# wengroup/matten

Hardware: AMD Instinct MI355X
Metric: edge_tensor_products_per_sec (higher is better)
Workload: dtype f32; 1 GPU; configs[2]: synthetic fcc-64 crystals (64 atoms, cutoff 5 A, 1152 edges each), paper hparams lmax=4, eval forward backbone+out_layer, one batch per step per GPU; last conv layer run for its live outputs only (258/842 radial-weight columns: the irreps its only reader takes) -- `value` counts 4 edge-TP per edge all the same, `value_full_layers` is the rate with the full last layer; nodes_per_gpu=64000, edges_per_gpu=1152000, conv_layers=4

## Files before the change

### include/matten_hip.h

```cpp
#ifndef MATTEN_HIP_H
#define MATTEN_HIP_H

#include <stddef.h>
#include <stdint.h>

#ifdef __cplusplus
extern "C" {
#endif

typedef void* matten_stream_t;

#define MATTEN_OK 0
#define MATTEN_EINVAL (-1)
#define MATTEN_ELAUNCH (-2)
#define MATTEN_ENOMEM (-3)

int matten_abi_version(void);

#define MATTEN_RADIAL_MAX_MID 3

size_t matten_csr_workspace_bytes(int64_t n_edges, int64_t n_nodes);
int matten_csr_counting_max_avg_degree(void);
int matten_csr_build(const int64_t* edge_index, int64_t n_edges, int64_t n_nodes, int32_t* perm,
                     int32_t* rowptr, int32_t* src_sorted, void* workspace, size_t workspace_bytes,
                     int32_t* err_flag, matten_stream_t stream);

int64_t matten_csr_split_bound(int64_t n_nodes, int64_t n_edges, int64_t max_len);
int matten_csr_split(const int32_t* rowptr, int64_t n_nodes, int64_t n_edges, int64_t max_len, int32_t* vrowptr,
                     int64_t* vseg, const float* num_neigh, float* vnn, matten_stream_t stream);

size_t matten_group_workspace_bytes(int64_t n, int64_t n_keys);
int matten_group_by_key(const int64_t* key, int64_t n, int64_t n_keys, int32_t* order, int32_t* seg,
                        void* workspace, size_t workspace_bytes, int32_t* err_flag, matten_stream_t stream);

int matten_species_embed(const int64_t* atomic_numbers, int64_t n_nodes, const int64_t* z_to_index,
                         int64_t min_z, int64_t max_z, int64_t n_species, const float* weight ,
                         const float* bias , int64_t dim, int64_t* species_index, int32_t* species_i32,
                         float* node_feats, float* node_attrs, int32_t* err_flag, matten_stream_t stream);

int matten_edge_geom(const float* pos, const int64_t* edge_index, const float* edge_cell_shift,
                     const float* cell, int64_t n_cells, const int64_t* batch, const int32_t* perm,
                     int64_t n_edges, int64_t n_nodes, int lmax, int n_basis, float r_start, float r_end,
                     float* geom_sorted, float* sh_sorted, int sh_stride, float* edge_vectors, float* edge_lengths,
                     float* edge_attrs, float* edge_embedding, matten_stream_t stream);

int matten_radial_mlp(const float* geom_sorted, int64_t n_edges, int n_basis, float r_start, float r_end,
                      const float* w0p, int nb_pad, const float* w1p, const float* w2p, int hidden, int w_pad,
                      float act_cst, void* w_edge, int out_is_bf16, matten_stream_t stream);
int matten_radial_mlp_deep(const float* geom_sorted, int64_t n_edges, int n_basis, float r_start, float r_end,
                           const float* w0p, int nb_pad, const float* w_mid, int n_mid, const float* w2p, int hidden,
                           int w_pad, float act_cst, void* w_edge, int out_is_bf16, matten_stream_t stream);

int matten_tp_tile_nodes(void);
int matten_tp_paths(const float* x, int64_t d_in, const void* w_edge, int64_t w_pad, const float* sh_sorted,
                    int64_t sh_dim, const int32_t* rowptr, const int32_t* src_sorted, int64_t n_nodes,
                    const int32_t* path_entries, const int32_t* unit_start, int64_t n_entries,
                    int64_t units_per_tile, int64_t d_mid, float avg_num_neighbors, const float* num_neigh,
                    float* agg , int w_is_bf16, matten_stream_t stream);

int matten_agg_linear_max_mt(void);
int matten_agg_linear_block_chunks(void);
size_t matten_agg_linear_lds_bytes(int64_t w_stride, int64_t n_io, int64_t n_blocks);
size_t matten_agg_linear_max_lds_bytes(void);
int matten_agg_linear(const float* agg, int64_t ld, const int32_t* order, const int32_t* seg, int64_t n_species,
                      const float* wtab, int64_t w_stride, const int32_t* io_table, int64_t n_io,
                      const int32_t* blocks, int64_t n_blocks, const float* add, int64_t add_ld, int64_t d_out,
                      int64_t n_rows, float* out, matten_stream_t stream);
int matten_agg_linear_gate(const float* agg, int64_t ld, const int32_t* order, const int32_t* seg, int64_t n_species,
                           const float* wtab, int64_t w_stride, const int32_t* io_table, int64_t n_io,
                           const int32_t* blocks, int64_t n_blocks, const float* add, int64_t add_ld, int64_t d_out,
                           int64_t n_rows, const int32_t* cmeta, const float* act_cst, const float* bn_scale,
                           const float* bn_shift, int64_t d_act, float* out, matten_stream_t stream);
int matten_agg_linear_gate_sets(void);
int matten_radial_hidden(const float* geom_sorted, int64_t n_edges, int n_basis, float r_start, float r_end,
                         const float* w0p, int nb_pad, const float* w1p, int hidden, uint16_t* h2s,
                         const float* h_scale, matten_stream_t stream);
int matten_radial_hidden_multi(const float* geom_sorted, int64_t n_edges, int n_basis, float r_start, float r_end,
                               const float* const* w0p, int nb_pad, const float* const* w1p, int hidden,
                               uint16_t* const* h2s, const float* const* h_scale, int n_layers,
                               matten_stream_t stream);
int matten_radial_hidden_deep(const float* geom_sorted, int64_t n_edges, int n_basis, float r_start, float r_end,
                              const float* w0p, int nb_pad, const float* w_mid, int n_mid, int hidden, uint16_t* h2s,
                              const float* h_scale, matten_stream_t stream);
int matten_radial_hidden_multi_deep(const float* geom_sorted, int64_t n_edges, int n_basis, float r_start, float r_end,
                                    const float* const* w0p, int nb_pad, const float* const* w_mid, int n_mid, int hidden,
                                    uint16_t* const* h2s, const float* const* h_scale, int n_layers,
                                    matten_stream_t stream);
int matten_tp_fused(const float* x, int64_t d_in, const uint16_t* h2s, const float* w2p, int64_t w_pad,
                    const float* sh_sorted, int64_t sh_stride, const int32_t* rowptr, const int32_t* src_sorted,
                    int64_t n_nodes, const int32_t* group_entries, const int32_t* unit_map, int64_t n_entries,
                    int64_t units_per_tile, int64_t lds_floats_per_wave, int64_t d_mid, float avg_num_neighbors,
                    const float* num_neigh, const uint16_t* a_split, const float* a_scale_inv,
                    float* agg , matten_stream_t stream);

int matten_tp_max_cols(void);
int matten_tp_max_cols_l0(void);
int matten_tp_max_cols_l1(void);
int matten_tp_groups_hash(void);

int matten_species_linear(const float* x, int64_t d_in, const int32_t* order, const int32_t* seg, int64_t n_species,
                          const float* wp, int64_t w_stride, const int32_t* segs, int64_t n_segs, int64_t d_out,
                          const float* add, int64_t add_ld, int64_t n_rows, float* out, matten_stream_t stream);

int matten_species_linear_rows(const float* x, int64_t d_in, const int32_t* order, const int32_t* seg, int64_t n_species,
                               const float* wp, int64_t w_stride, const int32_t* segs, int64_t n_segs, int64_t d_out,
                               const float* add, int64_t add_ld, int64_t n_rows, float* out, matten_stream_t stream);

int matten_gate_bn(const float* x, int64_t d_in, const int32_t* meta, int64_t d_out, const float* act_cst,
                   const float* running_mean, const float* running_var, const float* bn_weight,
                   const float* bn_bias, float eps, int64_t n_rows, float* out, matten_stream_t stream);

int matten_segment_reduce(const float* x, int64_t dim, const int64_t* ptr, int64_t n_segments, int mean,
                          float* out, matten_stream_t stream);
int matten_segment_minmax(const float* x, int64_t dim, const int64_t* ptr, int64_t n_segments, int take_max, float* out,
                          int64_t* arg, matten_stream_t stream);
int matten_segment_minmax_bwd(const float* dy, int64_t dim, const int64_t* arg, int64_t n_segments, float* dx,
                              matten_stream_t stream);

int64_t matten_radial_mlp_bwd_small_slices(int64_t n_edges);
int64_t matten_radial_mlp_bwd_w2_ranges(int64_t n_edges, int64_t w_pad);
int matten_radial_mlp_bwd(const float* geom_sorted, int64_t n_edges, int n_basis, float r_start, float r_end,
                          const float* w0p, int nb_pad, const float* w1p, const float* w2p, int hidden, int w_pad,
                          int w_cols, const void* dw, int64_t dw_ld, int dw_is_bf16, float* h2_scratch,
                          float* part_small, float* part_w2, float scale0, float scale1, float scale2,
                          float* grad_small, float* grad_w2, matten_stream_t stream);
int64_t matten_radial_mlp_bwd_w2_ranges_deep(int64_t n_edges, int64_t w_pad, int n_mid);
int matten_radial_mlp_bwd_deep(const float* geom_sorted, int64_t n_edges, int n_basis, float r_start, float r_end,
                               const float* w0p, int nb_pad, const float* w_mid, int n_mid, const float* w2p, int hidden,
                               int w_pad, int w_cols, const void* dw, int64_t dw_ld, int dw_is_bf16, float* h2_scratch,
                               float* part_small, float* part_w2, float scale0, float scale1, float scale2,
                               float* grad_small, float* grad_w2, matten_stream_t stream);
int matten_radial_pack(const float* w0, const float* w1, const float* w2, int n_basis, int nb_pad, int w_cols, int w_pad,
                       float scale0, float scale1, float scale2, float* w0p, float* w1p, float* w2p,
                       matten_stream_t stream);
int matten_radial_pack_deep(const float* w0, const float* w_mid, int n_mid, const float* w2, int n_basis, int nb_pad,
                            int w_cols, int w_pad, float scale0, float scale1, float scale2, float* w0p, float* w_mid_p,
                            float* w2p, matten_stream_t stream);
int matten_radial_pack_cols(const float* w0, const float* w1, const float* w2, int n_basis, int nb_pad, int w_cols,
                            const int64_t* cols, int n_cols, int w_pad, float scale0, float scale1, float scale2, float* w0p,
                            float* w1p, float* w2p, matten_stream_t stream);
int matten_radial_h_scale(const float* w0, const float* w1, int n_basis, float r_start, float r_end, float act_cst,
                          float* out2, matten_stream_t stream);
int matten_radial_pack_cols_deep(const float* w0, const float* w_mid, int n_mid, const float* w2, int n_basis, int nb_pad,
                                 int w_cols, const int64_t* cols, int n_cols, int w_pad, float scale0, float scale1,
                                 float scale2, float* w0p, float* w_mid_p, float* w2p, matten_stream_t stream);
int matten_radial_h_scale_deep(const float* w0, const float* w_mid, int n_mid, int n_basis, float r_start, float r_end,
                               float act_cst, float* out2, matten_stream_t stream);
int matten_split_a_tiles(const float* w2p, int64_t w_pad, const int32_t* group_entries, int64_t n_entries,
                         const float* h_scale, uint16_t* frag, float* scale_inv, matten_stream_t stream);
int matten_gather_scale(const float* src, const int64_t* idx, const float* scale, int64_t n, int64_t scale_period,
                        int scale_by_source, float* out, const int64_t* perm2, float* out2, matten_stream_t stream);
int64_t matten_species_linear_wgrad_scratch_floats(int64_t n_rows, int64_t n_species, int64_t w_stride);

int matten_dense_rows(const float* x, int64_t n_in, const float* q, int64_t n_out, int64_t n_rows, float* out,
                      matten_stream_t stream);



int matten_tp_backward(const float* x, int64_t d_in, const void* w_edge, int64_t w_ld, const float* sh_sorted,
                       int64_t sh_stride, const int32_t* src_sorted, const int32_t* dst_sorted,
                       const int32_t* col_meta, int64_t n_cols, const uint8_t* nnz_ijk, const float* nnz_c,
                       const float* g_agg, int64_t d_mid, float avg_num_neighbors, const float* num_neigh,
                       int64_t n_edges, float* dx, void* dw, int64_t dw_ld, const int32_t* in_ptr,
                       const int32_t* in_cols, int64_t n_in, int edge_is_bf16 ,
                       matten_stream_t stream);

int matten_adam_step(float* params, const float* grads, float* exp_avg, float* exp_avg_sq, int64_t n, const float* step,
                     float lr, float beta1, float beta2, float eps, float weight_decay, matten_stream_t stream);

int matten_tp_backward_lit(const float* x, int64_t d_in, const void* w_edge, int64_t w_ld, const float* sh_sorted,
                           int64_t sh_stride, const int32_t* src_sorted, const int32_t* dst_sorted, const int32_t* blocks,
                           int64_t n_blocks, int64_t max_mul, const int32_t* paths, int64_t n_paths, const float* g_agg,
                           int64_t d_mid, float avg_num_neighbors, const float* num_neigh, int64_t n_edges, float* dx,
                           void* dw, int64_t dw_ld, int edge_is_bf16, int64_t n_nodes, const int32_t* out_ptr,
                           const int32_t* out_perm, float* dx_edges, int max_l, matten_stream_t stream);
int matten_tp_backward_lit_wfree(const float* x, int64_t d_in, const uint16_t* h2s, const uint16_t* frag, const float* w_inv,
                                 const float* sh_sorted, int64_t sh_stride, const int32_t* src_sorted,
                                 const int32_t* dst_sorted, const int32_t* blocks, int64_t n_blocks, int64_t sum_lanes,
                                 const int32_t* paths, int64_t n_paths, const float* g_agg, int64_t d_mid,
                                 float avg_num_neighbors, const float* num_neigh, int64_t n_edges, float* dx, void* dw,
                                 int64_t dw_ld, int edge_is_bf16, int64_t n_nodes, const int32_t* out_ptr,
                                 const int32_t* out_perm, float* dx_edges, int64_t lds_floats, int max_l, int max_mul,
                                 matten_stream_t stream);

int matten_species_linear_wgrad(const float* x, int64_t d_in, const float* dy, int64_t d_out, const int32_t* order,
                                const int32_t* seg, int64_t n_species, int64_t n_rows, const int32_t* segs,
                                int64_t n_segs, int64_t w_stride, float* dwp, float* scratch, matten_stream_t stream);

int matten_gate_bwd(const float* x, int64_t d_in, const int32_t* meta, int64_t d_out, const float* act_cst,
                    const float* dy, int64_t n_rows, float* dx, matten_stream_t stream);

int64_t matten_bn_scratch_floats(int64_t n_rows, int64_t dim);
int matten_bn_train_fwd(const float* x, int64_t dim, int64_t n_rows, const int32_t* col2chan, const int32_t* chan,
                        int64_t n_chan, const float* weight, const float* bias, float eps, float* mean, float* nu,
                        float* y, float* running_mean, float* running_var, float momentum, float* scratch,
                        matten_stream_t stream);
int matten_bn_train_bwd(const float* x, const float* dy, int64_t dim, int64_t n_rows, const int32_t* col2chan,
                        const int32_t* chan, int64_t n_chan, const float* mean, const float* nu, const float* weight,
                        float eps, float* A, float* B, float* dx, float* dweight, float* dbias, float* scratch,
                        matten_stream_t stream);

int matten_norm_act(const float* x, int64_t dim, int64_t n_rows, const int32_t* chan, int64_t n_chan, int act,
                    float epsilon, const float* running_mean, const float* running_var, const float* bn_weight,
                    const float* bn_bias, float bn_eps, float* y, matten_stream_t stream);
int matten_norm_act_bwd(const float* x, const float* dy, int64_t dim, int64_t n_rows, const int32_t* chan, int64_t n_chan,
                        int act, float epsilon, float* dx, matten_stream_t stream);

int64_t matten_bn_eval_bwd_scratch_floats(int64_t n_rows, int64_t n_cols);
int matten_gate_bn_eval_bwd(const float* x, int64_t d_in, const int32_t* meta, int64_t d_out, const float* act_cst,
                            const int32_t* bn_chan, int64_t n_chan, const float* running_mean, const float* running_var,
                            const float* bn_weight, float eps, const float* dy, int64_t n_rows, float* dx, float* dweight,
                            float* dbias, float* scratch, matten_stream_t stream);
int matten_norm_act_bn_eval_bwd(const float* x, const float* dy, int64_t dim, int64_t n_rows, const int32_t* chan,
                                int64_t n_chan, int act, float epsilon, const float* running_mean,
                                const float* running_var, const float* bn_weight, float bn_eps, float* dx, float* dweight,
                                float* dbias, float* scratch, matten_stream_t stream);

int matten_instance_norm_fwd(const float* x, int64_t dim, int64_t n_rows, const int64_t* seg_ptr, const int64_t* seg_of_row,
                             int64_t n_seg, const int32_t* col2chan, const int32_t* chan, int64_t n_chan,
                             const float* weight, const float* bias, float eps, float* mean, float* nu, float* y,
                             matten_stream_t stream);
int matten_instance_norm_bwd(const float* x, const float* dy, int64_t dim, int64_t n_rows, const int64_t* seg_ptr,
                             const int64_t* seg_of_row, int64_t n_seg, const int32_t* col2chan, const int32_t* chan,
                             int64_t n_chan, const float* mean, const float* nu, const float* weight, float eps, float* A,
                             float* B, float* dx, matten_stream_t stream);

int matten_segment_reduce_bwd(const float* dy, int64_t dim, const int64_t* ptr, int64_t n_segments, int mean, float* dx,
                              matten_stream_t stream);


int matten_graph_prep(const double* pos, const double* cell, const int64_t* ptr, int64_t n_crystals, double r_cut,
                      double* frac, double* bound, int64_t* batch, float* pos_f32, float* cell_f32,
                      matten_stream_t stream);
int matten_neighbor_count(const double* pos, const double* cell, const int64_t* ptr, const double* frac,
                          const double* bound, const int64_t* pair_ptr, double r_cut, int64_t n_crystals,
                          int64_t max_atoms, int32_t* counts, int32_t* counts_t, matten_stream_t stream);
int matten_neighbor_summary(const int64_t* offsets, const int64_t* pair_ptr, int64_t n_crystals, int64_t* out2,
                            matten_stream_t stream);
int matten_neighbor_fill(const double* pos, const double* cell, const int64_t* ptr, const double* frac,
                         const double* bound, const int64_t* pair_ptr, double r_cut, int64_t n_crystals,
                         int64_t max_atoms, const int64_t* offsets, int64_t n_edges, int64_t* edge_index,
                         float* edge_cell_shift, float* num_neigh, const int64_t* offsets_t, int64_t n_atoms,
                         int32_t* rowptr, int32_t* src_sorted, int32_t* perm, matten_stream_t stream);

#ifdef __cplusplus
}
#endif
#endif
```

### matten_amd/_lib.py

```python
from __future__ import annotations

import ctypes
import os
from ctypes import c_float, c_int, c_int32, c_int64, c_size_t, c_void_p

_HERE = os.path.dirname(os.path.abspath(__file__))
LIB_PATH = os.path.join(_HERE, "libmatten_hip.so")

ABI_VERSION = 46

P = c_void_p
SIGNATURES = {
    "matten_abi_version": (c_int, []),
    "matten_csr_workspace_bytes": (c_size_t, [c_int64, c_int64]),
    "matten_group_workspace_bytes": (c_size_t, [c_int64, c_int64]),
    "matten_csr_counting_max_avg_degree": (c_int, []),
    "matten_csr_build": (c_int, [P, c_int64, c_int64, P, P, P, P, c_size_t, P, P]),
    "matten_csr_split_bound": (c_int64, [c_int64, c_int64, c_int64]),
    "matten_csr_split": (c_int, [P, c_int64, c_int64, c_int64, P, P, P, P, P]),
    "matten_group_by_key": (c_int, [P, c_int64, c_int64, P, P, P, c_size_t, P, P]),
    "matten_species_embed": (c_int, [P, c_int64, P, c_int64, c_int64, c_int64, P, P, c_int64, P, P, P, P, P, P]),
    "matten_edge_geom": (c_int, [P, P, P, P, c_int64, P, P, c_int64, c_int64, c_int, c_int, c_float, c_float, P, P, c_int, P, P, P, P, P]),
    "matten_radial_mlp": (c_int, [P, c_int64, c_int, c_float, c_float, P, c_int, P, P, c_int, c_int, c_float, P, c_int, P]),
    "matten_radial_mlp_deep": (c_int, [P, c_int64, c_int, c_float, c_float, P, c_int, P, c_int, P, c_int, c_int, c_float, P, c_int,
                                       P]),
    "matten_tp_tile_nodes": (c_int, []),
    "matten_tp_paths": (c_int, [P, c_int64, P, c_int64, P, c_int64, P, P, c_int64, P, P, c_int64, c_int64, c_int64, c_float, P, P, c_int,
                                P]),
    "matten_radial_hidden_multi": (c_int, [P, c_int64, c_int, c_float, c_float, P, c_int, P, c_int, P, P, c_int, P]),
    "matten_radial_hidden_multi_deep": (c_int, [P, c_int64, c_int, c_float, c_float, P, c_int, P, c_int, c_int, P, P, c_int, P]),
    "matten_agg_linear_max_mt": (c_int, []),
    "matten_agg_linear_block_chunks": (c_int, []),
    "matten_agg_linear_lds_bytes": (c_size_t, [c_int64, c_int64, c_int64]),
    "matten_agg_linear_max_lds_bytes": (c_size_t, []),
    "matten_agg_linear": (c_int, [P, c_int64, P, P, c_int64, P, c_int64, P, c_int64, P, c_int64, P, c_int64, c_int64,
                                  c_int64, P, P]),
    "matten_agg_linear_gate": (c_int, [P, c_int64, P, P, c_int64, P, c_int64, P, c_int64, P, c_int64, P, c_int64, c_int64,
                                       c_int64, P, P, P, P, c_int64, P, P]),
    "matten_agg_linear_gate_sets": (c_int, []),
    "matten_radial_hidden": (c_int, [P, c_int64, c_int, c_float, c_float, P, c_int, P, c_int, P, P, P]),
    "matten_radial_hidden_deep": (c_int, [P, c_int64, c_int, c_float, c_float, P, c_int, P, c_int, c_int, P, P, P]),
    "matten_tp_max_cols": (c_int, []),
    "matten_tp_max_cols_l0": (c_int, []),
    "matten_tp_max_cols_l1": (c_int, []),
    "matten_tp_groups_hash": (c_int, []),
    "matten_tp_fused": (c_int, [P, c_int64, P, P, c_int64, P, c_int64, P, P, c_int64, P, P, c_int64, c_int64, c_int64, c_int64, c_float, P, P, P, P, P]),
    "matten_species_linear": (c_int, [P, c_int64, P, P, c_int64, P, c_int64, P, c_int64, c_int64, P, c_int64, c_int64, P, P]),
    "matten_species_linear_rows": (c_int, [P, c_int64, P, P, c_int64, P, c_int64, P, c_int64, c_int64, P, c_int64, c_int64, P, P]),
    "matten_radial_mlp_bwd_small_slices": (c_int64, [c_int64]),
    "matten_radial_mlp_bwd_w2_ranges": (c_int64, [c_int64, c_int64]),
    "matten_radial_mlp_bwd_w2_ranges_deep": (c_int64, [c_int64, c_int64, c_int]),
    "matten_radial_mlp_bwd": (c_int, [P, c_int64, c_int, c_float, c_float, P, c_int, P, P, c_int, c_int, c_int, P, c_int64,
                                      c_int, P, P, P, c_float, c_float, c_float, P, P, P]),
    "matten_radial_mlp_bwd_deep": (c_int, [P, c_int64, c_int, c_float, c_float, P, c_int, P, c_int, P, c_int, c_int, c_int, P,
                                           c_int64, c_int, P, P, P, c_float, c_float, c_float, P, P, P]),
    "matten_radial_pack": (c_int, [P, P, P, c_int, c_int, c_int, c_int, c_float, c_float, c_float, P, P, P, P]),
    "matten_radial_pack_deep": (c_int, [P, P, c_int, P, c_int, c_int, c_int, c_int, c_float, c_float, c_float, P, P, P, P]),
    "matten_radial_pack_cols": (c_int, [P, P, P, c_int, c_int, c_int, P, c_int, c_int, c_float, c_float, c_float, P, P, P, P]),
    "matten_radial_pack_cols_deep": (c_int, [P, P, c_int, P, c_int, c_int, c_int, P, c_int, c_int, c_float, c_float, c_float, P, P,
                                             P, P]),
    "matten_radial_h_scale": (c_int, [P, P, c_int, c_float, c_float, c_float, P, P]),
    "matten_radial_h_scale_deep": (c_int, [P, P, c_int, c_int, c_float, c_float, c_float, P, P]),
    "matten_split_a_tiles": (c_int, [P, c_int64, P, c_int64, P, P, P, P]),
    "matten_gather_scale": (c_int, [P, P, P, c_int64, c_int64, c_int, P, P, P, P]),
    "matten_species_linear_wgrad_scratch_floats": (c_int64, [c_int64, c_int64, c_int64]),
    "matten_tp_backward": (c_int, [P, c_int64, P, c_int64, P, c_int64, P, P, P, c_int64, P, P, P, c_int64, c_float, P, c_int64, P, P, c_int64,
                                   P, P, c_int64, c_int, P]),
    "matten_tp_backward_lit": (c_int, [P, c_int64, P, c_int64, P, c_int64, P, P, P, c_int64, c_int64, P, c_int64, P, c_int64, c_float,
                                       P, c_int64, P, P, c_int64, c_int, c_int64, P, P, P, c_int, P]),
    "matten_tp_backward_lit_wfree": (c_int, [P, c_int64, P, P, P, P, c_int64, P, P, P, c_int64, c_int64, P, c_int64, P, c_int64, c_float,
                                             P, c_int64, P, P, c_int64, c_int, c_int64, P, P, P, c_int64, c_int, c_int, P]),
    "matten_adam_step": (c_int, [P, P, P, P, c_int64, P, c_float, c_float, c_float, c_float, c_float, P]),
    "matten_species_linear_wgrad": (c_int, [P, c_int64, P, c_int64, P, P, c_int64, c_int64, P, c_int64, c_int64, P, P, P]),
    "matten_gate_bwd": (c_int, [P, c_int64, P, c_int64, P, P, c_int64, P, P]),
    "matten_bn_scratch_floats": (c_int64, [c_int64, c_int64]),
    "matten_bn_train_fwd": (c_int, [P, c_int64, c_int64, P, P, c_int64, P, P, c_float, P, P, P, P, P, c_float, P, P]),
    "matten_bn_train_bwd": (c_int, [P, P, c_int64, c_int64, P, P, c_int64, P, P, P, c_float, P, P, P, P, P, P, P]),
    "matten_norm_act": (c_int, [P, c_int64, c_int64, P, c_int64, c_int, c_float, P, P, P, P, c_float, P, P]),
    "matten_norm_act_bwd": (c_int, [P, P, c_int64, c_int64, P, c_int64, c_int, c_float, P, P]),
    "matten_bn_eval_bwd_scratch_floats": (c_int64, [c_int64, c_int64]),
    "matten_gate_bn_eval_bwd": (c_int, [P, c_int64, P, c_int64, P, P, c_int64, P, P, P, c_float, P, c_int64, P, P, P, P, P]),
    "matten_norm_act_bn_eval_bwd": (c_int, [P, P, c_int64, c_int64, P, c_int64, c_int, c_float, P, P, P, c_float, P, P, P, P,
                                            P]),
    "matten_instance_norm_fwd": (c_int, [P, c_int64, c_int64, P, P, c_int64, P, P, c_int64, P, P, c_float, P, P, P, P]),
    "matten_instance_norm_bwd": (c_int, [P, P, c_int64, c_int64, P, P, c_int64, P, P, c_int64, P, P, P, c_float, P, P, P, P]),
    "matten_segment_reduce_bwd": (c_int, [P, c_int64, P, c_int64, c_int, P, P]),
    "matten_graph_prep": (c_int, [P, P, P, c_int64, ctypes.c_double, P, P, P, P, P, P]),
    "matten_neighbor_count": (c_int, [P, P, P, P, P, P, ctypes.c_double, c_int64, c_int64, P, P, P]),
    "matten_neighbor_summary": (c_int, [P, P, c_int64, P, P]),
    "matten_neighbor_fill": (c_int, [P, P, P, P, P, P, ctypes.c_double, c_int64, c_int64, P, c_int64, P, P, P, P, c_int64,
                                     P, P, P, P]),
    "matten_gate_bn": (c_int, [P, c_int64, P, c_int64, P, P, P, P, P, c_float, c_int64, P, P]),
    "matten_segment_reduce": (c_int, [P, c_int64, P, c_int64, c_int, P, P]),
    "matten_segment_minmax": (c_int, [P, c_int64, P, c_int64, c_int, P, P, P]),
    "matten_segment_minmax_bwd": (c_int, [P, c_int64, P, c_int64, P, P]),
    "matten_dense_rows": (c_int, [P, c_int64, P, c_int64, c_int64, P, P]),
}

_lib = None


class MattenHipError(RuntimeError):
    pass


def load() -> ctypes.CDLL:
    global _lib
    if _lib is not None:
        return _lib
    if not os.path.exists(LIB_PATH):
        raise MattenHipError(
            f"{LIB_PATH} not found: the HIP extension is not built. matten_amd has no CPU fallback; "
            "run `make -C matten_amd/csrc` (needs hipcc, --offload-arch=gfx950)."
        )
    lib = ctypes.CDLL(LIB_PATH)
    for name, (res, args) in SIGNATURES.items():
        try:
            fn = getattr(lib, name)
        except AttributeError as e:
            raise MattenHipError(f"symbol {name} missing from {LIB_PATH}") from e
        fn.restype = res
        fn.argtypes = args
    v = lib.matten_abi_version()
    if v != ABI_VERSION:
        raise MattenHipError(f"ABI version mismatch: library {v}, python binding {ABI_VERSION}")
    _lib = lib
    return lib


_ERRORS = {-1: "MATTEN_EINVAL (bad argument)", -2: "MATTEN_ELAUNCH (HIP launch failed)", -3: "MATTEN_ENOMEM (workspace too small)"}


def check(rc: int, what: str) -> None:
    if rc != 0:
        raise MattenHipError(f"{what} failed: {_ERRORS.get(rc, rc)}")
```

### matten_amd/csrc/csr.hip

```cpp
#include <cstring>

#include <rocprim/device/device_radix_sort.hpp>
#include <rocprim/device/device_scan.hpp>

#include "common.h"

namespace {

__global__ void csr_keys_kernel(const int64_t* __restrict__ edge_index, int64_t E, int64_t N,
                                int32_t* __restrict__ keys, int32_t* __restrict__ vals, int32_t* err_flag) {
    int64_t e = (int64_t)blockIdx.x * blockDim.x + threadIdx.x;
    if (e >= E) return;
    int64_t s = edge_index[e];
    int64_t d = edge_index[E + e];
    if (s < 0 || s >= N || d < 0 || d >= N) {
        atomicOr(err_flag, 1);
        d = d < 0 ? 0 : (d >= N ? N - 1 : d);
    }
    keys[e] = (int32_t)d;
    vals[e] = (int32_t)e;
}

__global__ void csr_rowptr_kernel(const int32_t* __restrict__ keys_sorted, int64_t E, int64_t N,
                                  int32_t* __restrict__ rowptr) {
    int64_t n = (int64_t)blockIdx.x * blockDim.x + threadIdx.x;
    if (n > N) return;
    int64_t lo = 0, hi = E;
    while (lo < hi) {
        int64_t mid = (lo + hi) >> 1;
        if (keys_sorted[mid] < (int32_t)n) lo = mid + 1; else hi = mid;
    }
    rowptr[n] = (int32_t)lo;
}

__global__ void csr_src_kernel(const int64_t* __restrict__ edge_index, const int32_t* __restrict__ perm, int64_t E,
                               int64_t N, int32_t* __restrict__ src_sorted) {
    int64_t e = (int64_t)blockIdx.x * blockDim.x + threadIdx.x;
    if (e >= E) return;
    int64_t s = edge_index[perm[e]];
    s = s < 0 ? 0 : (s >= N ? N - 1 : s);
    src_sorted[e] = (int32_t)s;
}

__global__ void zero_i32_kernel(int32_t* __restrict__ p, int64_t n) {
    int64_t i = (int64_t)blockIdx.x * blockDim.x + threadIdx.x;
    if (i < n) p[i] = 0;
}

__global__ void csr_count_kernel(const int64_t* __restrict__ edge_index, int64_t E, int64_t N,
                                 int32_t* __restrict__ deg, int32_t* __restrict__ slot, int32_t* err_flag) {
    int64_t e = (int64_t)blockIdx.x * blockDim.x + threadIdx.x;
    if (e >= E) return;
    int64_t s = edge_index[e];
    int64_t d = edge_index[E + e];
    if (s < 0 || s >= N || d < 0 || d >= N) {
        atomicOr(err_flag, 1);
        d = d < 0 ? 0 : (d >= N ? N - 1 : d);
    }
    slot[e] = atomicAdd(&deg[d], 1);
}

__global__ void csr_place_kernel(const int64_t* __restrict__ edge_index, int64_t E, int64_t N,
                                 const int32_t* __restrict__ rowptr, const int32_t* __restrict__ slot,
                                 int32_t* __restrict__ ids) {
    int64_t e = (int64_t)blockIdx.x * blockDim.x + threadIdx.x;
    if (e >= E) return;
    int64_t d = edge_index[E + e];
    d = d < 0 ? 0 : (d >= N ? N - 1 : d);
    ids[rowptr[d] + slot[e]] = (int32_t)e;
}

constexpr int CSR_HUB_DEGREE = 2048;
constexpr int CSR_HUB_THREADS = 1024;
constexpr int CSR_HUB_BLOCKS = 64;

__global__ void csr_rank_kernel(const int64_t* __restrict__ edge_index, const int32_t* __restrict__ rowptr,
                                const int32_t* __restrict__ ids, int64_t E, int64_t N, int32_t* __restrict__ perm,
                                int32_t* __restrict__ src_sorted, int32_t* __restrict__ hubs) {
    const int64_t node = ((int64_t)blockIdx.x * blockDim.x + threadIdx.x) >> 4;
    if (node >= N) return;
    const int sub = threadIdx.x & 15;
    const int beg = rowptr[node], d = rowptr[node + 1] - beg;
    if (d > CSR_HUB_DEGREE) {
        if (sub == 0) hubs[atomicAdd(&hubs[N], 1)] = (int32_t)node;
        return;
    }
    for (int i = sub; i < d; i += 16) {
        const int id = ids[beg + i];
        int rank = 0;
        int j = 0;
        for (; j + 8 <= d; j += 8) {
            int v[8];
#pragma unroll
            for (int q = 0; q < 8; ++q) v[q] = ids[beg + j + q];
#pragma unroll
            for (int q = 0; q < 8; ++q) rank += v[q] < id;
        }
        for (; j < d; ++j) rank += ids[beg + j] < id;
        perm[beg + rank] = id;
        int64_t s = edge_index[id];
        s = s < 0 ? 0 : (s >= N ? N - 1 : s);
        src_sorted[beg + rank] = (int32_t)s;
    }
}

__global__ __launch_bounds__(CSR_HUB_THREADS) void csr_hub_kernel(const int64_t* __restrict__ edge_index,
                                                                  const int32_t* __restrict__ rowptr, int32_t* ids,
                                                                  int64_t N, int32_t* __restrict__ perm,
                                                                  int32_t* __restrict__ src_sorted,
                                                                  const int32_t* __restrict__ hubs) {
    const int n_hubs = hubs[N];
    for (int h = blockIdx.x; h < n_hubs; h += gridDim.x) {
        const int node = hubs[h];
        const int beg = rowptr[node], d = rowptr[node + 1] - beg;
        int32_t* a = ids + beg;
        for (int64_t k = 2; (k >> 1) < d; k <<= 1) {
            for (int64_t j = k >> 1; j > 0; j >>= 1) {
                const int64_t m = (j == (k >> 1)) ? k - 1 : j;
                for (int64_t i = threadIdx.x; i < d; i += CSR_HUB_THREADS) {
                    const int64_t l = i ^ m;
                    if (l > i && l < d) {
                        const int32_t x = a[i], y = a[l];
                        if (y < x) a[i] = y, a[l] = x;
                    }
                }
                __syncthreads();
            }
        }
        for (int64_t i = threadIdx.x; i < d; i += CSR_HUB_THREADS) {
            const int32_t id = a[i];
            perm[beg + i] = id;
            int64_t s = edge_index[id];
            s = s < 0 ? 0 : (s >= N ? N - 1 : s);
            src_sorted[beg + i] = (int32_t)s;
        }
        __syncthreads();
    }
}

__global__ void group_keys_kernel(const int64_t* __restrict__ key, int64_t n, int64_t n_keys,
                                  int32_t* __restrict__ keys, int32_t* __restrict__ vals, int32_t* err_flag) {
    int64_t i = (int64_t)blockIdx.x * blockDim.x + threadIdx.x;
    if (i >= n) return;
    int64_t k = key[i];
    if (k < 0 || k >= n_keys) {
        atomicOr(err_flag, 1);
        k = k < 0 ? 0 : n_keys - 1;
    }
    keys[i] = (int32_t)k;
    vals[i] = (int32_t)i;
}

constexpr int GROUP_COUNTING_MAX_KEYS = 256;
constexpr int GROUP_WAVES = 4;

__device__ __forceinline__ int group_key_of(const int64_t* __restrict__ key, int64_t i, int64_t n, int64_t n_keys,
                                            int32_t* err_flag) {
    if (i >= n) return -1;
    int64_t k = key[i];
    if (k < 0 || k >= n_keys) {
        atomicOr(err_flag, 1);
        k = k < 0 ? 0 : n_keys - 1;
    }
    return (int)k;
}

__global__ __launch_bounds__(GROUP_WAVES * 64) void group_hist_kernel(const int64_t* __restrict__ key, int64_t n,
                                                                      int64_t n_keys, int64_t n_runs,
                                                                      int32_t* __restrict__ cnt, int32_t* err_flag) {
    __shared__ int h[GROUP_WAVES][GROUP_COUNTING_MAX_KEYS];
    const int wv = threadIdx.x >> 6, lane = threadIdx.x & 63;
    const int64_t run = (int64_t)blockIdx.x * GROUP_WAVES + wv;
    for (int kk = lane; kk < n_keys; kk += 64) h[wv][kk] = 0;
    __builtin_amdgcn_wave_barrier();
    const int k = group_key_of(key, run * 64 + lane, n, n_keys, err_flag);
    if (k >= 0) atomicAdd(&h[wv][k], 1);
    __builtin_amdgcn_s_waitcnt(0xc07f);
    __builtin_amdgcn_wave_barrier();
    if (run < n_runs)
        for (int kk = lane; kk < n_keys; kk += 64) cnt[(int64_t)kk * n_runs + run] = h[wv][kk];
}

__global__ __launch_bounds__(GROUP_WAVES * 64) void group_place_kernel(const int64_t* __restrict__ key, int64_t n,
                                                                       int64_t n_keys, int64_t n_runs,
                                                                       const int32_t* __restrict__ offs,
                                                                       int32_t* __restrict__ order,
                                                                       int32_t* __restrict__ seg, int32_t* err_flag) {
    const int lane = threadIdx.x & 63;
    const int64_t i = (int64_t)blockIdx.x * blockDim.x + threadIdx.x;
    const int64_t run = i >> 6;
    if (i <= n_keys) seg[i] = i < n_keys ? offs[i * n_runs] : (int32_t)n;
    const int k = group_key_of(key, i, n, n_keys, err_flag);
    unsigned long long todo = __ballot(k >= 0);
    int rank = 0;
    while (todo) {
        const int kf = __shfl(k, __ffsll((long long)todo) - 1);
        const unsigned long long m = __ballot(k == kf);
        if (k == kf) rank = __popcll(m & ((1ull << lane) - 1ull));
        todo &= ~m;
    }
    if (k >= 0) order[offs[(int64_t)k * n_runs + run] + rank] = (int32_t)i;
}

inline size_t align256(size_t x) { return (x + 255) & ~(size_t)255; }

inline int key_bits(int64_t N) {
    int b = 1;
    while (((int64_t)1 << b) < N && b < 31) ++b;
    return b;
}

}

__global__ __launch_bounds__(1024) void csr_split_kernel(const int* __restrict__ rowptr, int N, int max_len, int nv_bound,
                                                         int* __restrict__ vrowptr, int64_t* __restrict__ vseg,
                                                         const float* __restrict__ num_neigh, float* __restrict__ vnn) {
    __shared__ int sh[1024];
    __shared__ int carry_s;
    const int t = threadIdx.x;
    if (t == 0) carry_s = 0;
    __syncthreads();
    const int E = rowptr[N];
    for (int base = 0; base < N; base += 1024) {
        const int n = base + t;
        int beg = 0, k = 0, d = 0;
        if (n < N) {
            beg = rowptr[n];
            d = rowptr[n + 1] - beg;
            k = max(1, (d + max_len - 1) / max_len);
        }
        sh[t] = k;
        __syncthreads();
        for (int off = 1; off < 1024; off <<= 1) {
            const int v = t >= off ? sh[t - off] : 0;
            __syncthreads();
            sh[t] += v;
            __syncthreads();
        }
        const int carry = carry_s;
        const int first = carry + sh[t] - k;
        if (n < N) {
            vseg[n] = first;
            for (int i = 0; i < k; ++i) {
                const int v = first + i;
                if (v < nv_bound) {
                    vrowptr[v] = beg + (int)((int64_t)i * d / k);
                    if (vnn) vnn[v] = num_neigh[n];
                }
            }
        }
        __syncthreads();
        if (t == 1023) carry_s = carry + sh[1023];
        __syncthreads();
    }
    const int nv = min(carry_s, nv_bound);
    if (t == 0) vseg[N] = nv;
    for (int v = nv + t; v <= nv_bound; v += 1024) {
        vrowptr[v] = E;
        if (vnn && v < nv_bound) vnn[v] = 1.0f;
    }
}

extern "C" size_t matten_csr_workspace_bytes(int64_t E, int64_t N) {
    if (E < 0 || N < 0) return 0;
    size_t tmp = 0;
    int32_t* p = nullptr;
    (void)rocprim::radix_sort_pairs(nullptr, tmp, p, p, p, p, (size_t)(E > 0 ? E : 1), 0, key_bits(N), 0, false);
    size_t scan_tmp = 0;
    (void)rocprim::exclusive_scan(nullptr, scan_tmp, p, p, 0, (size_t)(N + 1), rocprim::plus<int32_t>());
    return 3 * align256((size_t)(E > 0 ? E : 1) * sizeof(int32_t)) + align256(tmp) + align256((size_t)(N + 1) * sizeof(int32_t)) +
           align256(scan_tmp) + 256;
}

extern "C" size_t matten_group_workspace_bytes(int64_t n, int64_t n_keys) {
    if (n < 0 || n_keys <= 0) return 0;
    size_t need = matten_csr_workspace_bytes(n, n_keys);
    if (n_keys <= GROUP_COUNTING_MAX_KEYS) {
        const size_t table = (size_t)n_keys * (size_t)((n + 63) / 64 + 1);
        size_t scan_tmp = 0;
        int32_t* p = nullptr;
        (void)rocprim::exclusive_scan(nullptr, scan_tmp, p, p, 0, table, rocprim::plus<int32_t>());
        const size_t counting = 2 * align256(table * sizeof(int32_t)) + align256(scan_tmp) + 256;
        if (counting > need) need = counting;
    }
    return need;
}

constexpr int64_t CSR_COUNTING_MAX_AVG_DEGREE = 64;

extern "C" int matten_csr_counting_max_avg_degree(void) { return (int)CSR_COUNTING_MAX_AVG_DEGREE; }

extern "C" int matten_csr_build(const int64_t* edge_index, int64_t E, int64_t N, int32_t* perm, int32_t* rowptr,
                                int32_t* src_sorted, void* workspace, size_t workspace_bytes, int32_t* err_flag,
                                matten_stream_t stream_) {
    hipStream_t stream = (hipStream_t)stream_;
    if (E < 0 || N < 0 || N >= ((int64_t)1 << 31) || E >= ((int64_t)1 << 31)) return MATTEN_EINVAL;
    if (!rowptr || !err_flag) return MATTEN_EINVAL;
    if (E == 0) {
        zero_i32_kernel<<<(unsigned)matten_cdiv(N + 1, 256), 256, 0, stream>>>(rowptr, N + 1);
        MATTEN_LAUNCH_CHECK();
        return MATTEN_OK;
    }
    if (!edge_index || !perm || !src_sorted || !workspace) return MATTEN_EINVAL;
    size_t need = matten_csr_workspace_bytes(E, N);
    if (workspace_bytes < need) return MATTEN_ENOMEM;

    char* ws = (char*)workspace;
    size_t seg = align256((size_t)E * sizeof(int32_t));
    int32_t* keys_in = (int32_t*)ws;
    int32_t* keys_out = (int32_t*)(ws + seg);
    int32_t* vals_in = (int32_t*)(ws + 2 * seg);
    void* tmp = ws + 3 * seg;
    size_t tmp_bytes = workspace_bytes - 3 * seg;

    const int T = 256;
    if (N > 0 && E <= CSR_COUNTING_MAX_AVG_DEGREE * N) {
        int32_t* ids = (int32_t*)ws;
        int32_t* slot = (int32_t*)(ws + seg);
        int32_t* deg = (int32_t*)(ws + 2 * seg);
        const size_t deg_bytes = align256((size_t)(N + 1) * sizeof(int32_t));
        void* scan_tmp = ws + 2 * seg + deg_bytes;
        size_t scan_bytes = workspace_bytes - 2 * seg - deg_bytes;
        zero_i32_kernel<<<(unsigned)matten_cdiv(N + 1, T), T, 0, stream>>>(deg, N + 1);
        MATTEN_LAUNCH_CHECK();
        csr_count_kernel<<<(unsigned)matten_cdiv(E, T), T, 0, stream>>>(edge_index, E, N, deg, slot, err_flag);
        MATTEN_LAUNCH_CHECK();
        if (rocprim::exclusive_scan(scan_tmp, scan_bytes, deg, rowptr, 0, (size_t)(N + 1), rocprim::plus<int32_t>(),
                                    stream) != hipSuccess)
            return MATTEN_ELAUNCH;
        csr_place_kernel<<<(unsigned)matten_cdiv(E, T), T, 0, stream>>>(edge_index, E, N, rowptr, slot, ids);
        MATTEN_LAUNCH_CHECK();
        csr_rank_kernel<<<(unsigned)matten_cdiv(N * 16, T), T, 0, stream>>>(edge_index, rowptr, ids, E, N, perm,
                                                                           src_sorted, deg);
        MATTEN_LAUNCH_CHECK();
        if (E > CSR_HUB_DEGREE) {
            const int64_t max_hubs = E / CSR_HUB_DEGREE;
            csr_hub_kernel<<<(unsigned)(max_hubs < CSR_HUB_BLOCKS ? max_hubs : CSR_HUB_BLOCKS), CSR_HUB_THREADS, 0,
                             stream>>>(edge_index, rowptr, ids, N, perm, src_sorted, deg);
            MATTEN_LAUNCH_CHECK();
        }
        return MATTEN_OK;
    }
    csr_keys_kernel<<<(unsigned)matten_cdiv(E, T), T, 0, stream>>>(edge_index, E, N, keys_in, vals_in, err_flag);
    MATTEN_LAUNCH_CHECK();
    if (rocprim::radix_sort_pairs(tmp, tmp_bytes, keys_in, keys_out, vals_in, perm, (size_t)E, 0, key_bits(N), stream,
                                  false) != hipSuccess)
        return MATTEN_ELAUNCH;
    csr_rowptr_kernel<<<(unsigned)matten_cdiv(N + 1, T), T, 0, stream>>>(keys_out, E, N, rowptr);
    MATTEN_LAUNCH_CHECK();
    csr_src_kernel<<<(unsigned)matten_cdiv(E, T), T, 0, stream>>>(edge_index, perm, E, N, src_sorted);
    MATTEN_LAUNCH_CHECK();
    return MATTEN_OK;
}

extern "C" int matten_group_by_key(const int64_t* key, int64_t n, int64_t n_keys, int32_t* order, int32_t* seg,
                                   void* workspace, size_t workspace_bytes, int32_t* err_flag, matten_stream_t stream_) {
    hipStream_t stream = (hipStream_t)stream_;
    if (n < 0 || n_keys <= 0 || n_keys >= ((int64_t)1 << 31) || n >= ((int64_t)1 << 31)) return MATTEN_EINVAL;
    if (!seg || !err_flag) return MATTEN_EINVAL;
    if (n == 0) {
        zero_i32_kernel<<<(unsigned)matten_cdiv(n_keys + 1, 256), 256, 0, stream>>>(seg, n_keys + 1);
        MATTEN_LAUNCH_CHECK();
        return MATTEN_OK;
    }
    if (!key || !order || !workspace) return MATTEN_EINVAL;
    if (workspace_bytes < matten_group_workspace_bytes(n, n_keys)) return MATTEN_ENOMEM;
    char* ws = (char*)workspace;
    if (n_keys <= GROUP_COUNTING_MAX_KEYS) {
        const int64_t n_runs = (n + 63) / 64;
        const size_t table = (size_t)n_keys * (size_t)n_runs;
        const size_t tb = align256((size_t)n_keys * (size_t)(n_runs + 1) * sizeof(int32_t));
        int32_t* cnt = (int32_t*)ws;
        int32_t* offs = (int32_t*)(ws + tb);
        void* scan_tmp = ws + 2 * tb;
        size_t scan_bytes = workspace_bytes - 2 * tb;
        const int TB = GROUP_WAVES * 64;
        group_hist_kernel<<<(unsigned)matten_cdiv(n_runs, GROUP_WAVES), TB, 0, stream>>>(key, n, n_keys, n_runs, cnt,
                                                                                        err_flag);
        MATTEN_LAUNCH_CHECK();
        if (rocprim::exclusive_scan(scan_tmp, scan_bytes, cnt, offs, 0, table, rocprim::plus<int32_t>(), stream) !=
            hipSuccess)
            return MATTEN_ELAUNCH;
        const int64_t threads = n > n_keys + 1 ? n : n_keys + 1;
        group_place_kernel<<<(unsigned)matten_cdiv(threads, TB), TB, 0, stream>>>(key, n, n_keys, n_runs, offs, order,
                                                                                 seg, err_flag);
        MATTEN_LAUNCH_CHECK();
        return MATTEN_OK;
    }
    size_t sg = align256((size_t)n * sizeof(int32_t));
    int32_t* keys_in = (int32_t*)ws;
    int32_t* keys_out = (int32_t*)(ws + sg);
    int32_t* vals_in = (int32_t*)(ws + 2 * sg);
    void* tmp = ws + 3 * sg;
    size_t tmp_bytes = workspace_bytes - 3 * sg;
    const int T = 256;
    group_keys_kernel<<<(unsigned)matten_cdiv(n, T), T, 0, stream>>>(key, n, n_keys, keys_in, vals_in, err_flag);
    MATTEN_LAUNCH_CHECK();
    if (rocprim::radix_sort_pairs(tmp, tmp_bytes, keys_in, keys_out, vals_in, order, (size_t)n, 0, key_bits(n_keys),
                                  stream, false) != hipSuccess)
        return MATTEN_ELAUNCH;
    csr_rowptr_kernel<<<(unsigned)matten_cdiv(n_keys + 1, T), T, 0, stream>>>(keys_out, n, n_keys, seg);
    MATTEN_LAUNCH_CHECK();
    return MATTEN_OK;
}

extern "C" int64_t matten_csr_split_bound(int64_t n_nodes, int64_t n_edges, int64_t max_len) {
    return max_len > 0 ? n_nodes + n_edges / max_len : n_nodes;
}

extern "C" int matten_csr_split(const int32_t* rowptr, int64_t n_nodes, int64_t n_edges, int64_t max_len, int32_t* vrowptr,
                                int64_t* vseg, const float* num_neigh, float* vnn, matten_stream_t stream_) {
    if (n_nodes < 0 || n_edges < 0 || max_len <= 0 || n_nodes >= ((int64_t)1 << 30) || n_edges >= ((int64_t)1 << 31))
        return MATTEN_EINVAL;
    if (!rowptr || !vrowptr || !vseg || ((num_neigh == nullptr) != (vnn == nullptr))) return MATTEN_EINVAL;
    const int64_t bound = matten_csr_split_bound(n_nodes, n_edges, max_len);
    if (bound >= ((int64_t)1 << 31)) return MATTEN_EINVAL;
    csr_split_kernel<<<1, 1024, 0, (hipStream_t)stream_>>>(rowptr, (int)n_nodes, (int)max_len, (int)bound, vrowptr, vseg,
                                                          num_neigh, vnn);
    MATTEN_LAUNCH_CHECK();
    return MATTEN_OK;
}
```

### matten_amd/csrc/edge.hip

```cpp
#include "common.h"
#include "sh.h"

namespace {

constexpr int SH_TILE_RS = 36;

template <int LMAX>
__global__ __launch_bounds__(256) void edge_geom_kernel(const float* __restrict__ pos, const int64_t* __restrict__ edge_index,
                                 const float* __restrict__ shift, const float* __restrict__ cell, int64_t n_cells,
                                 const int64_t* __restrict__ batch, const int32_t* __restrict__ perm, int64_t E,
                                 int64_t N, int n_basis, float r_start, float r_end, float4* __restrict__ geom_sorted,
                                 float* __restrict__ sh_sorted, int sh_stride, float* __restrict__ edge_vectors,
                                 float* __restrict__ edge_lengths, float* __restrict__ edge_attrs,
                                 float* __restrict__ edge_embedding) {
    constexpr int SH = (LMAX + 1) * (LMAX + 1);
    __shared__ __attribute__((aligned(16))) float sh_tile[4 * 64 * SH_TILE_RS];
    const int64_t e_raw = (int64_t)blockIdx.x * blockDim.x + threadIdx.x;
    if (e_raw - (threadIdx.x & 63) >= E) return;
    const bool live = e_raw < E;
    const int64_t e = live ? e_raw : E - 1;
    int64_t o = perm ? (int64_t)perm[e] : e;
    int64_t i = edge_index[o];
    int64_t j = edge_index[E + o];
    i = i < 0 ? 0 : (i >= N ? N - 1 : i);
    j = j < 0 ? 0 : (j >= N ? N - 1 : j);
    float vx = pos[3 * j + 0] - pos[3 * i + 0];
    float vy = pos[3 * j + 1] - pos[3 * i + 1];
    float vz = pos[3 * j + 2] - pos[3 * i + 2];
    if (cell) {
        int64_t b = (n_cells > 1 && batch) ? batch[i] : 0;
        b = b < 0 ? 0 : (b >= n_cells ? n_cells - 1 : b);
        const float* c = cell + 9 * b;
        float s0 = shift[3 * o + 0], s1 = shift[3 * o + 1], s2 = shift[3 * o + 2];
        vx += s0 * c[0] + s1 * c[3] + s2 * c[6];
        vy += s0 * c[1] + s1 * c[4] + s2 * c[7];
        vz += s0 * c[2] + s1 * c[5] + s2 * c[8];
    }
    float len = sqrtf(vx * vx + vy * vy + vz * vz);
    if (live) geom_sorted[e] = make_float4(vx, vy, vz, len);

    float y[SH];
    matten::real_sh<LMAX>(vx, vy, vz, len, y);
    if (sh_stride == 32) {
        float* tile = sh_tile + (threadIdx.x >> 6) * (64 * SH_TILE_RS);
        const int lane = threadIdx.x & 63;
#pragma unroll
        for (int q = 0; q < 8; ++q)
            *reinterpret_cast<float4*>(tile + lane * SH_TILE_RS + 4 * q) =
                make_float4(4 * q < SH ? y[4 * q < SH ? 4 * q : 0] : 0.0f,
                            4 * q + 1 < SH ? y[4 * q + 1 < SH ? 4 * q + 1 : 0] : 0.0f,
                            4 * q + 2 < SH ? y[4 * q + 2 < SH ? 4 * q + 2 : 0] : 0.0f,
                            4 * q + 3 < SH ? y[4 * q + 3 < SH ? 4 * q + 3 : 0] : 0.0f);
        __builtin_amdgcn_s_waitcnt(0xc07f);
        __builtin_amdgcn_wave_barrier();
        const int64_t e0 = e_raw - lane;
        const int64_t n_here = E - e0 < 64 ? E - e0 : 64;
        float4* dst = reinterpret_cast<float4*>(sh_sorted + e0 * 32);
#pragma unroll
        for (int i = 0; i < 8; ++i) {
            const int f = i * 64 + lane;
            if ((f >> 3) < n_here)
                dst[f] = *reinterpret_cast<const float4*>(tile + (f >> 3) * SH_TILE_RS + 4 * (f & 7));
        }
    } else if (live) {
#pragma unroll
        for (int k = 0; k < SH; ++k) sh_sorted[e * sh_stride + k] = y[k];
        for (int k = SH; k < sh_stride; ++k) sh_sorted[e * sh_stride + k] = 0.0f;
    }
    if (!live) return;

    if (edge_vectors) {
        edge_vectors[3 * o + 0] = vx;
        edge_vectors[3 * o + 1] = vy;
        edge_vectors[3 * o + 2] = vz;
    }
    if (edge_lengths) edge_lengths[o] = len;
    if (edge_attrs) {
#pragma unroll
        for (int k = 0; k < SH; ++k) edge_attrs[o * SH + k] = y[k];
    }
    if (edge_embedding) {
        for (int k = 0; k < n_basis; ++k)
            edge_embedding[o * n_basis + k] = matten::bessel_basis(len, k, n_basis, r_start, r_end);
    }
}

__global__ void species_embed_kernel(const int64_t* __restrict__ Z, int64_t N, const int64_t* __restrict__ lut,
                                     int64_t min_z, int64_t max_z, int64_t S, const float* __restrict__ W,
                                     const float* __restrict__ b, int64_t dim, int64_t* __restrict__ species_index,
                                     int32_t* __restrict__ species_i32, float* __restrict__ feats,
                                     float* __restrict__ attrs, int32_t* err_flag) {
    int64_t n = (int64_t)blockIdx.x * blockDim.y + threadIdx.y;
    if (n >= N) return;
    int64_t z = Z[n];
    int64_t idx = -1;
    if (z < min_z || z > max_z) {
        if (threadIdx.x == 0) atomicOr(err_flag, 2);
    } else {
        idx = lut[z - min_z];
        if (idx < 0 || idx >= S) {
            if (threadIdx.x == 0) atomicOr(err_flag, 4);
            idx = -1;
        }
    }
    if (threadIdx.x == 0) {
        if (species_index) species_index[n] = idx;
        if (species_i32) species_i32[n] = (int32_t)(idx < 0 ? 0 : idx);
    }
    int64_t s = idx < 0 ? 0 : idx;
    for (int64_t d = threadIdx.x; d < dim; d += blockDim.x) feats[n * dim + d] = W[d * S + s] + b[d];
    if (attrs)
        for (int64_t c = threadIdx.x; c < S; c += blockDim.x) attrs[n * S + c] = (c == idx) ? 1.0f : 0.0f;
}

}

extern "C" int matten_species_embed(const int64_t* atomic_numbers, int64_t n_nodes, const int64_t* z_to_index,
                                    int64_t min_z, int64_t max_z, int64_t n_species, const float* weight,
                                    const float* bias, int64_t dim, int64_t* species_index, int32_t* species_i32,
                                    float* node_feats, float* node_attrs, int32_t* err_flag,
                                    matten_stream_t stream_) {
    hipStream_t stream = (hipStream_t)stream_;
    if (n_nodes < 0 || dim <= 0 || n_species <= 0) return MATTEN_EINVAL;
    if (n_nodes == 0) return MATTEN_OK;
    if (!atomic_numbers || !z_to_index || !weight || !bias || !node_feats || !err_flag) return MATTEN_EINVAL;
    dim3 block(16, 16);
    species_embed_kernel<<<(unsigned)matten_cdiv(n_nodes, 16), block, 0, stream>>>(
        atomic_numbers, n_nodes, z_to_index, min_z, max_z, n_species, weight, bias, dim, species_index, species_i32,
        node_feats, node_attrs, err_flag);
    MATTEN_LAUNCH_CHECK();
    return MATTEN_OK;
}

extern "C" int matten_edge_geom(const float* pos, const int64_t* edge_index, const float* edge_cell_shift,
                                const float* cell, int64_t n_cells, const int64_t* batch, const int32_t* perm,
                                int64_t n_edges, int64_t n_nodes, int lmax, int n_basis, float r_start, float r_end,
                                float* geom_sorted, float* sh_sorted, int sh_stride, float* edge_vectors, float* edge_lengths,
                                float* edge_attrs, float* edge_embedding, matten_stream_t stream_) {
    hipStream_t stream = (hipStream_t)stream_;
    if (n_edges < 0 || n_nodes < 0 || (n_edges > 0 && n_nodes == 0) || lmax < 0 || lmax > 4 || n_basis < 0 || sh_stride < (lmax + 1) * (lmax + 1)) return MATTEN_EINVAL;
    if (n_edges == 0) return MATTEN_OK;
    if (!pos || !edge_index || !geom_sorted || !sh_sorted) return MATTEN_EINVAL;
    if (cell && !edge_cell_shift) return MATTEN_EINVAL;
    const int T = 256;
    unsigned grid = (unsigned)matten_cdiv(n_edges, T);
#define LAUNCH(L)                                                                                              \
    edge_geom_kernel<L><<<grid, T, 0, stream>>>(pos, edge_index, edge_cell_shift, cell, n_cells, batch, perm,  \
                                                n_edges, n_nodes, n_basis, r_start, r_end, (float4*)geom_sorted, \
                                                sh_sorted, sh_stride, edge_vectors, edge_lengths, edge_attrs, edge_embedding)
    switch (lmax) {
        case 0: LAUNCH(0); break;
        case 1: LAUNCH(1); break;
        case 2: LAUNCH(2); break;
        case 3: LAUNCH(3); break;
        default: LAUNCH(4); break;
    }
#undef LAUNCH
    MATTEN_LAUNCH_CHECK();
    return MATTEN_OK;
}
```

### matten_amd/nn/_nequip.py

```python
from typing import Union

import torch

from .. import ops
from ..data.irreps import DataKey, ModuleIrreps
from ..o3 import Irreps


def with_batch(data: DataKey.Type) -> DataKey.Type:
    if DataKey.BATCH not in data:
        pos = data[DataKey.POSITIONS]
        data[DataKey.BATCH] = torch.zeros(len(pos), dtype=torch.long, device=pos.device)
    return data


def ensure_graph(data: DataKey.Type, err=None) -> DataKey.Type:
    if DataKey.AMD_ROWPTR not in data:
        n_nodes = data[DataKey.POSITIONS].shape[0]
        perm, rowptr, src, err = ops.csr_build(data[DataKey.EDGE_INDEX], n_nodes, err=err)
        data[DataKey.AMD_PERM], data[DataKey.AMD_ROWPTR], data[DataKey.AMD_SRC] = perm, rowptr, src
        data["_amd_csr_err"] = err
    return data


def ensure_edge_geometry(data: DataKey.Type, lmax: int = None, want_vectors=False, want_lengths=False,
                         want_attrs=False, want_embedding=False) -> DataKey.Type:
    have = DataKey.AMD_GEOM in data
    missing = (
        (want_vectors and DataKey.EDGE_VECTORS not in data)
        or (want_lengths and DataKey.EDGE_LENGTH not in data)
        or (want_attrs and DataKey.EDGE_ATTRS not in data)
        or (want_embedding and DataKey.EDGE_EMBEDDING not in data)
    )
    if have and not missing:
        return data
    ensure_graph(data)
    if lmax is None:
        lmax = int(data["_amd_lmax"]) if "_amd_lmax" in data else 0
    data["_amd_lmax"] = lmax
    nb, r0, r1 = 0, 0.0, 1.0
    if DataKey.AMD_RBF in data:
        nb, r0, r1 = data[DataKey.AMD_RBF].tolist()
        nb = int(nb)
    out = ops.edge_geom(
        data[DataKey.POSITIONS], data[DataKey.EDGE_INDEX], data.get(DataKey.EDGE_CELL_SHIFT),
        data.get(DataKey.CELL), data.get(DataKey.BATCH), data[DataKey.AMD_PERM], lmax, nb, r0, r1,
        want_vectors=want_vectors, want_lengths=want_lengths, want_attrs=want_attrs,
        want_embedding=want_embedding and nb > 0,
    )
    data[DataKey.AMD_GEOM], data[DataKey.AMD_SH] = out["geom_sorted"], out["sh_sorted"]
    for key, name in ((DataKey.EDGE_VECTORS, "edge_vectors"), (DataKey.EDGE_LENGTH, "edge_lengths"),
                      (DataKey.EDGE_ATTRS, "edge_attrs"), (DataKey.EDGE_EMBEDDING, "edge_embedding")):
        if out[name] is not None:
            data[key] = out[name]
    return data


def ensure_training_edge_tensors(data: DataKey.Type) -> DataKey.Type:
    if "_amd_dst_sorted" not in data:
        ensure_edge_geometry(data)
        perm = data[DataKey.AMD_PERM].long()
        data["_amd_dst_sorted"] = data[DataKey.EDGE_INDEX][1][perm].to(torch.int32).contiguous()
        src = data[DataKey.AMD_SRC].long()
        pairs = torch.stack([src, src])
        out_perm, out_ptr, _, _ = ops.csr_build(pairs, int(data[DataKey.POSITIONS].shape[0]))
        data["_amd_out_csr"] = (out_ptr, out_perm)
    return data


def with_edge_vectors(data: DataKey.Type, with_lengths: bool = True) -> DataKey.Type:
    return ensure_edge_geometry(data, want_vectors=True, want_lengths=with_lengths)


class SphericalHarmonicEdgeAttrs(ModuleIrreps, torch.nn.Module):
    out_field: str

    def __init__(
        self,
        irreps_edge_sh: Union[int, str, Irreps],
        edge_sh_normalization: str = "component",
        edge_sh_normalize: bool = True,
        irreps_in=None,
        out_field: str = DataKey.EDGE_ATTRS,
        materialize: bool = False,
    ):
        super().__init__()
        self.out_field = out_field
        if isinstance(irreps_edge_sh, int):
            self.irreps_edge_sh = Irreps.spherical_harmonics(irreps_edge_sh)
        else:
            self.irreps_edge_sh = Irreps(irreps_edge_sh)
        lmax = len(self.irreps_edge_sh) - 1
        if self.irreps_edge_sh != Irreps.spherical_harmonics(lmax) or lmax > 4:
            raise NotImplementedError(f"edge SH must be 0e+1o+...+lmax (lmax<=4), got {self.irreps_edge_sh}")
        if edge_sh_normalization != "component" or not edge_sh_normalize:
            raise NotImplementedError("only normalize=True, normalization='component' (the reference default)")
        self.lmax = lmax
        self.materialize = materialize
        self.init_irreps(irreps_in=irreps_in, irreps_out={out_field: self.irreps_edge_sh})

    def forward(self, data: DataKey.Type) -> DataKey.Type:
        ensure_edge_geometry(data, lmax=self.lmax, want_vectors=self.materialize, want_attrs=self.materialize)
        if self.materialize and self.out_field != DataKey.EDGE_ATTRS:
            data[self.out_field] = data[DataKey.EDGE_ATTRS]
        return data
```

### matten_amd/nn/embedding.py

```python
from typing import Dict, List, Tuple

import numpy as np
import torch

from .. import ops
from ..data.irreps import DataKey, ModuleIrreps
from ..o3 import Irreps


class _AtomicNumberToIndex(torch.nn.Module):

    def __init__(self, allowed_atomic_numbers: List[int]):
        super().__init__()
        allowed = torch.as_tensor(sorted(allowed_atomic_numbers), dtype=torch.long)
        lut = torch.full((int(allowed.max() - allowed.min()) + 1,), -1, dtype=torch.long)
        lut[allowed - allowed.min()] = torch.arange(len(allowed), dtype=torch.long)
        self.register_buffer("_min_Z", allowed.min())
        self.register_buffer("_max_Z", allowed.max())
        self.register_buffer("_num_species", torch.as_tensor(len(allowed)))
        self.register_buffer("_Z_to_index", lut)
        self._host = (int(allowed.min()), int(allowed.max()), len(allowed))
        self._allowed = [int(z) for z in allowed]

    @property
    def num_species(self):
        return self._num_species

    def raise_for_flags(self, flags: int, atomic_numbers: torch.Tensor):
        if flags & 2:
            raise RuntimeError(
                "Invalid atomic numbers. Expect atomic numbers to be in the range "
                f"[{self._host[0]}, {self._host[1]}], but got min {int(atomic_numbers.min())} "
                f"and max {int(atomic_numbers.max())}"
            )
        if flags & 4:
            z = atomic_numbers.cpu()
            for i, n in enumerate(z.tolist()):
                if n not in self._allowed:
                    raise RuntimeError(
                        f"Expect atomic numbers to be in {self._allowed}, "
                        f"got invalid atomic numbers `{n}` for data point `{i}`."
                    )

    def forward(self, atomic_numbers: torch.Tensor) -> torch.Tensor:
        lo, hi, _ = self._host
        if atomic_numbers.min() < lo or atomic_numbers.max() > hi:
            self.raise_for_flags(2, atomic_numbers)
        index = self._Z_to_index[atomic_numbers - lo]
        if index.min() < 0:
            self.raise_for_flags(4, atomic_numbers)
        return index


class SpeciesEmbedding(ModuleIrreps, torch.nn.Module):
    def __init__(
        self,
        irreps_in: Dict[str, Irreps] = None,
        embedding_dim: int = 16,
        num_species: int = None,
        allowed_species: List[int] = None,
        out_fields: Tuple[str] = (DataKey.NODE_ATTRS, DataKey.NODE_FEATURES),
        use_atom_feats: bool = False,
        atom_feats_dim: int = None,
        materialize: bool = False,
        check_species: bool = True,
    ):
        super().__init__()
        if allowed_species is not None and num_species is not None:
            raise ValueError("allowed_species and num_species cannot both be provided.")
        if allowed_species is None:
            raise NotImplementedError("matten_amd needs `allowed_species` (every shipped config provides it)")
        if use_atom_feats and atom_feats_dim is None:
            raise ValueError("`atom_feats_dim` must be provided if `use_atom_feats` is True.")
        self.use_atom_feats = use_atom_feats
        self.embedding_dim = embedding_dim
        self.out_fields = out_fields
        self.materialize = materialize
        self.check_species = check_species
        self.atomic_number_to_index = _AtomicNumberToIndex(allowed_species)
        self.num_species = len(allowed_species)
        self.init_irreps(
            irreps_in,
            {DataKey.NODE_ATTRS: Irreps(f"{self.num_species}x0e"),
             DataKey.NODE_FEATURES: Irreps(f"{embedding_dim + (atom_feats_dim if use_atom_feats else 0)}x0e")},
        )
        self.linear = torch.nn.Linear(self.num_species, embedding_dim)

    def finish_checks(self) -> None:
        pending, self._pending = getattr(self, "_pending", None), None
        if pending is None:
            return
        ev, host, Z, n_nodes = pending
        ev.synchronize()
        self._raise_for(host.tolist(), Z, n_nodes)

    def _raise_for(self, flags, Z, n_nodes) -> None:
        if flags[0]:
            self.atomic_number_to_index.raise_for_flags(flags[0], Z)
        if flags[1] & 1:
            rng = f"[0, {n_nodes})" if n_nodes is not None else "the batch's node range"
            raise IndexError(f"edge_index holds node ids outside {rng} (a malformed batch)")

    def raise_for_last_flags(self, n_nodes=None) -> None:
        flags_dev = getattr(self, "_last_flags", None)
        if flags_dev is None:
            return
        self._raise_for(flags_dev.tolist(), self._last_Z, n_nodes)

    def forward(self, data: DataKey.Type) -> DataKey.Type:
        a2i = self.atomic_number_to_index
        lo, hi, S = a2i._host
        if DataKey.SPECIES_INDEX in data:
            Z = data[DataKey.SPECIES_INDEX]
            lut = torch.arange(S, dtype=torch.int64, device=Z.device)
            lo, hi = 0, S - 1
            provided = True
        elif DataKey.ATOMIC_NUMBERS in data:
            Z, lut, provided = data[DataKey.ATOMIC_NUMBERS], a2i._Z_to_index, False
        else:
            raise ValueError("Nothing in `data` to encode. Need either species_index or atomic_numbers")
        flags_dev = torch.zeros(3, dtype=torch.int32, device=Z.device)
        sidx, s32, feats, attrs, _ = ops.species_embed(
            Z, lut, lo, hi, S, self.linear.weight, self.linear.bias, want_attrs=self.materialize, err=flags_dev[0:1]
        )
        if DataKey.EDGE_INDEX in data:
            from ._nequip import ensure_graph

            built_here = DataKey.AMD_ROWPTR not in data
            csr_err = ensure_graph(data, err=flags_dev[1:2]).get("_amd_csr_err")
            if not built_here and csr_err is not None:
                flags_dev[1:2] = csr_err
        order, seg, _ = ops.group_by_key(sidx, S, err=flags_dev[2:3])
        self._last_flags, self._last_Z = flags_dev, Z
        n_nodes = data[DataKey.POSITIONS].shape[0] if DataKey.POSITIONS in data else None
        if self.check_species == "deferred":
            self.finish_checks()
            host = torch.empty(3, dtype=torch.int32, pin_memory=True)
            host.copy_(flags_dev, non_blocking=True)
            ev = torch.cuda.Event()
            ev.record(torch.cuda.current_stream(Z.device))
            self._pending = (ev, host, Z, n_nodes)
        elif self.check_species:
            self.raise_for_last_flags(n_nodes)
        if not provided:
            data[DataKey.SPECIES_INDEX] = sidx
        data[DataKey.AMD_SPECIES] = (order, seg)
        data[DataKey.AMD_SPECIES_I32] = s32
        if attrs is not None:
            data[DataKey.NODE_ATTRS] = attrs
        if torch.is_grad_enabled() and self.linear.weight.requires_grad:
            from ..autograd import SpeciesEmbedFn

            if self.__dict__.get("_wgrad_segs") is None:
                from ._tables import DeviceTables

                dim = self.linear.weight.shape[0]
                self.__dict__["_wgrad_segs"] = DeviceTables(segs=np.array([[0, 1, 1, 0, dim, 0, 0, 0]], dtype=np.int32))
            feats = SpeciesEmbedFn.apply(self.linear.weight, self.linear.bias, feats, (order, seg),
                                         self._wgrad_segs.get("segs", feats.device))
        if self.use_atom_feats:
            extra = data["atom_feats"]
            if extra.dim() != 2 or extra.shape[0] != feats.shape[0]:
                raise ValueError(f"atom_feats must be [n_atoms, atom_feats_dim], got {tuple(extra.shape)}")
            feats = torch.cat([feats, extra.to(feats.dtype)], dim=1)
        data[DataKey.NODE_FEATURES] = feats
        return data


class EdgeLengthEmbedding(ModuleIrreps, torch.nn.Module):
    REQUIRED_KEYS_IRREPS_IN = [DataKey.POSITIONS, DataKey.EDGE_INDEX]

    def __init__(
        self,
        irreps_in: Dict[str, Irreps] = None,
        out_field: str = DataKey.EDGE_EMBEDDING,
        num_basis: int = 10,
        start: float = 0.0,
        end: float = 5.0,
        basis: str = "bessel",
        cutoff: bool = True,
        materialize: bool = False,
    ):
        super().__init__()
        if basis != "bessel" or not cutoff:
            raise NotImplementedError("matten_amd implements the Bessel basis with cutoff (all shipped configs)")
        self.num_basis, self.start, self.end, self.basis, self.cutoff = num_basis, start, end, basis, cutoff
        self.out_field = out_field
        self.materialize = materialize
        self.init_irreps(irreps_in, irreps_out={out_field: Irreps(f"{num_basis}x0e")})

    def forward(self, data: DataKey.Type) -> DataKey.Type:
        from ._nequip import ensure_edge_geometry

        data[DataKey.AMD_RBF] = torch.tensor([self.num_basis, self.start, self.end], dtype=torch.float64)
        if self.materialize:
            ensure_edge_geometry(data, want_lengths=True, want_embedding=True)
        return data
```

### matten_amd/ops.py

```python
from __future__ import annotations

from typing import Optional, Tuple

import os

import numpy as np

import torch

from . import _lib
from .nn._tables import bump_weights_epoch


_EVENTS = None
_EVENTS_ONLY = None


def enable_event_timing(flag: bool = True, only=None) -> None:
    global _EVENTS, _EVENTS_ONLY
    _EVENTS = {} if flag else None
    _EVENTS_ONLY = tuple(only) if (flag and only) else None


def event_timings_ms():
    if _EVENTS is None:
        return {}
    return {k: [a.elapsed_time(b) for a, b in v] for k, v in _EVENTS.items()}


class _timed:
    def __init__(self, name: str):
        self.name = name

    def __enter__(self):
        self.on = _EVENTS is not None and (_EVENTS_ONLY is None or self.name.startswith(_EVENTS_ONLY))
        if self.on:
            self.a = torch.cuda.Event(enable_timing=True)
            self.a.record(torch.cuda.current_stream())
        return self

    def __exit__(self, *exc):
        if self.on and _EVENTS is not None:
            b = torch.cuda.Event(enable_timing=True)
            b.record(torch.cuda.current_stream())
            _EVENTS.setdefault(self.name, []).append((self.a, b))
        return False


SH_STRIDE = 32


def _ptr(t: Optional[torch.Tensor]):
    return None if t is None else t.data_ptr()


_raw_stream = getattr(torch._C, "_cuda_getCurrentRawStream", None)


def _stream() -> int:
    if _raw_stream is not None:
        return _raw_stream(torch.cuda.current_device())
    return torch.cuda.current_stream().cuda_stream


def _need(t: torch.Tensor, dtype, name: str) -> torch.Tensor:
    if not isinstance(t, torch.Tensor):
        raise TypeError(f"{name}: expected a tensor, got {type(t)}")
    if not t.is_cuda:
        raise _lib.MattenHipError(
            f"{name} is on {t.device}: matten_amd runs on MI355X only (no CPU fallback). Move the batch to cuda."
        )
    if t.dtype != dtype:
        raise TypeError(f"{name}: expected dtype {dtype}, got {t.dtype}")
    return t if t.is_contiguous() else t.contiguous()


def _need_rows(t: torch.Tensor, dtype, name: str) -> torch.Tensor:
    if isinstance(t, torch.Tensor) and t.dim() == 2 and t.stride(1) == 1 and t.stride(0) >= t.shape[1] and t.is_cuda \
            and t.dtype == dtype:
        return t
    return _need(t, dtype, name)


def _err_flag(err, dev) -> torch.Tensor:
    if err is None:
        return torch.zeros(1, dtype=torch.int32, device=dev)
    if err.dtype != torch.int32 or err.numel() != 1 or err.device != dev:
        raise ValueError("err must be an int32 tensor of one element on the inputs' device")
    return err


def csr_build(edge_index: torch.Tensor, n_nodes: int, err: torch.Tensor = None) -> Tuple[torch.Tensor, torch.Tensor, torch.Tensor, torch.Tensor]:
    lib = _lib.load()
    edge_index = _need(edge_index, torch.int64, "edge_index")
    E = edge_index.shape[1]
    dev = edge_index.device
    perm = torch.empty(E, dtype=torch.int32, device=dev)
    rowptr = torch.empty(n_nodes + 1, dtype=torch.int32, device=dev)
    src = torch.empty(E, dtype=torch.int32, device=dev)
    err = _err_flag(err, dev)
    nbytes = lib.matten_csr_workspace_bytes(E, n_nodes)
    ws = torch.empty(max(nbytes, 1), dtype=torch.uint8, device=dev)
    _lib.check(
        lib.matten_csr_build(_ptr(edge_index), E, n_nodes, _ptr(perm), _ptr(rowptr), _ptr(src), _ptr(ws), nbytes,
                             _ptr(err), _stream()),
        "matten_csr_build",
    )
    return perm, rowptr, src, err


def csr_split(rowptr: torch.Tensor, n_edges: int, max_len: int, num_neigh: torch.Tensor = None):
    lib = _lib.load()
    rowptr = _need(rowptr, torch.int32, "rowptr")
    N = rowptr.shape[0] - 1
    bound = int(lib.matten_csr_split_bound(N, n_edges, max_len))
    dev = rowptr.device
    vrowptr = torch.empty(bound + 1, dtype=torch.int32, device=dev)
    vseg = torch.empty(N + 1, dtype=torch.int64, device=dev)
    vnn = None
    if num_neigh is not None:
        num_neigh = _need(num_neigh, torch.float32, "num_neigh")
        vnn = torch.empty(bound, dtype=torch.float32, device=dev)
    _lib.check(lib.matten_csr_split(_ptr(rowptr), N, n_edges, max_len, _ptr(vrowptr), _ptr(vseg), _ptr(num_neigh), _ptr(vnn),
                                    _stream()), "matten_csr_split")
    return vrowptr, vseg, vnn


def group_by_key(key: torch.Tensor, n_keys: int, err: torch.Tensor = None) -> Tuple[torch.Tensor, torch.Tensor, torch.Tensor]:
    lib = _lib.load()
    key = _need(key, torch.int64, "key")
    n = key.shape[0]
    dev = key.device
    order = torch.empty(n, dtype=torch.int32, device=dev)
    seg = torch.empty(n_keys + 1, dtype=torch.int32, device=dev)
    err = _err_flag(err, dev)
    nbytes = lib.matten_group_workspace_bytes(n, n_keys)
    ws = torch.empty(max(nbytes, 1), dtype=torch.uint8, device=dev)
    _lib.check(lib.matten_group_by_key(_ptr(key), n, n_keys, _ptr(order), _ptr(seg), _ptr(ws), nbytes, _ptr(err),
                                       _stream()), "matten_group_by_key")
    return order, seg, err


def species_embed(atomic_numbers, z_to_index, min_z: int, max_z: int, n_species: int, weight, bias,
                  want_attrs: bool = False, err: torch.Tensor = None):
    lib = _lib.load()
    Z = _need(atomic_numbers, torch.int64, "atomic_numbers")
    lut = _need(z_to_index, torch.int64, "_Z_to_index")
    W = _need(weight, torch.float32, "linear.weight")
    b = _need(bias, torch.float32, "linear.bias")
    N, dim = Z.shape[0], W.shape[0]
    dev = Z.device
    sidx = torch.empty(N, dtype=torch.int64, device=dev)
    s32 = torch.empty(N, dtype=torch.int32, device=dev)
    feats = torch.empty(N, dim, dtype=torch.float32, device=dev)
    attrs = torch.empty(N, n_species, dtype=torch.float32, device=dev) if want_attrs else None
    err = _err_flag(err, dev)
    _lib.check(
        lib.matten_species_embed(_ptr(Z), N, _ptr(lut), min_z, max_z, n_species, _ptr(W), _ptr(b), dim, _ptr(sidx),
                                 _ptr(s32), _ptr(feats), _ptr(attrs), _ptr(err), _stream()),
        "matten_species_embed",
    )
    return sidx, s32, feats, attrs, err


def edge_geom(pos, edge_index, edge_cell_shift, cell, batch, perm, lmax: int, n_basis: int = 0, r_start: float = 0.0,
              r_end: float = 1.0, want_vectors=False, want_lengths=False, want_attrs=False, want_embedding=False):
    lib = _lib.load()
    pos = _need(pos, torch.float32, "pos")
    edge_index = _need(edge_index, torch.int64, "edge_index")
    E = edge_index.shape[1]
    dev = pos.device
    n_cells = 0
    if cell is not None:
        cell = _need(cell, torch.float32, "cell").reshape(-1, 3, 3)
        n_cells = cell.shape[0]
        edge_cell_shift = _need(edge_cell_shift, torch.float32, "edge_cell_shift")
        if n_cells > 1:
            batch = _need(batch, torch.int64, "batch")
    sh_dim = (lmax + 1) ** 2
    geom = torch.empty(E, 4, dtype=torch.float32, device=dev)
    sh = torch.empty(E, SH_STRIDE, dtype=torch.float32, device=dev)
    out = {"geom_sorted": geom, "sh_sorted": sh}
    ev = torch.empty(E, 3, dtype=torch.float32, device=dev) if want_vectors else None
    el = torch.empty(E, dtype=torch.float32, device=dev) if want_lengths else None
    ea = torch.empty(E, sh_dim, dtype=torch.float32, device=dev) if want_attrs else None
    ee = torch.empty(E, n_basis, dtype=torch.float32, device=dev) if want_embedding else None
    _lib.check(
        lib.matten_edge_geom(_ptr(pos), _ptr(edge_index), _ptr(edge_cell_shift), _ptr(cell), n_cells, _ptr(batch),
                             _ptr(perm), E, pos.shape[0], lmax, n_basis, r_start, r_end, _ptr(geom), _ptr(sh), SH_STRIDE, _ptr(ev),
                             _ptr(el),
                             _ptr(ea), _ptr(ee), _stream()),
        "matten_edge_geom",
    )
    out.update(edge_vectors=ev, edge_lengths=el, edge_attrs=ea, edge_embedding=ee)
    return out


def _edge_dtype(t: torch.Tensor, name: str) -> torch.Tensor:
    if not isinstance(t, torch.Tensor) or t.dtype not in (torch.float32, torch.bfloat16):
        raise TypeError(f"{name}: expected an fp32 or bf16 tensor")
    return _need(t, t.dtype, name)


def radial_mlp(geom_sorted, n_basis: int, r_start: float, r_end: float, w0p, w1p, w2p, out_dtype=torch.float32) -> torch.Tensor:
    lib = _lib.load()
    geom_sorted = _need(geom_sorted, torch.float32, "geom_sorted")
    w0p, w1p, w2p = (_need(w, torch.float32, n) for w, n in ((w0p, "w0p"), (w1p, "w1p"), (w2p, "w2p")))
    E = geom_sorted.shape[0]
    nb_pad, hidden = w0p.shape
    w_pad = w2p.shape[1]
    if out_dtype not in (torch.float32, torch.bfloat16):
        raise TypeError("radial_mlp: out_dtype must be fp32 or bf16")
    out = torch.empty(E, w_pad, dtype=out_dtype, device=geom_sorted.device)
    with _timed(f"radial_mlp/w_pad={w_pad}"):
        rc = lib.matten_radial_mlp(_ptr(geom_sorted), E, n_basis, r_start, r_end, _ptr(w0p), nb_pad, _ptr(w1p),
                                   _ptr(w2p), hidden, w_pad, 1.0, _ptr(out), int(out_dtype == torch.bfloat16), _stream())
    _lib.check(rc, "matten_radial_mlp")
    return out


def radial_pack(w0, w1, w2, scales):
    lib = _lib.load()
    w0, w1, w2 = (_need(w, torch.float32, n) for w, n in ((w0, "layer0.weight"), (w1, "layer1.weight"), (w2, "layer2.weight")))
    nb, h = w0.shape
    W = w2.shape[1]
    nb_pad, w_pad = (nb + 3) // 4 * 4, (W + 15) // 16 * 16
    dev = w0.device
    w0p = torch.empty(nb_pad, h, dtype=torch.float32, device=dev)
    w1p = torch.empty(h, h, dtype=torch.float32, device=dev)
    w2p = torch.empty(h, w_pad, dtype=torch.float32, device=dev)
    _lib.check(lib.matten_radial_pack(_ptr(w0), _ptr(w1), _ptr(w2), nb, nb_pad, W, w_pad, float(scales[0]), float(scales[1]),
                                      float(scales[2]), _ptr(w0p), _ptr(w1p), _ptr(w2p), _stream()), "matten_radial_pack")
    return w0p, w1p, w2p


def fused_operands(w0, w1, w2, scales, cols, group_entries, n_tiles: int, r_start: float, r_end: float, act_cst: float):
    lib = _lib.load()
    w0, w1, w2 = (_need(w, torch.float32, n) for w, n in ((w0, "layer0.weight"), (w1, "layer1.weight"), (w2, "layer2.weight")))
    cols = _need(cols, torch.int64, "fused_cols")
    group_entries = _need(group_entries, torch.int32, "group_entries")
    nb, h = w0.shape
    W, n_cols = w2.shape[1], cols.numel()
    nb_pad, w_pad = (nb + 3) // 4 * 4, (n_cols + 15) // 16 * 16 + 16
    dev = w0.device
    w0p = torch.empty(nb_pad, h, dtype=torch.float32, device=dev)
    w1p = torch.empty(h, h, dtype=torch.float32, device=dev)
    w2p = torch.empty(h, w_pad, dtype=torch.float32, device=dev)
    hs = torch.empty(2, dtype=torch.float32, device=dev)
    n_ent = group_entries.shape[0]
    frag = torch.empty(n_tiles, 64, 16, dtype=torch.float16, device=dev)
    inv = torch.empty(n_ent, dtype=torch.float32, device=dev)
    st = _stream()
    _lib.check(lib.matten_radial_pack_cols(_ptr(w0), _ptr(w1), _ptr(w2), nb, nb_pad, W, _ptr(cols), n_cols, w_pad,
                                           float(scales[0]), float(scales[1]), float(scales[2]), _ptr(w0p), _ptr(w1p),
                                           _ptr(w2p), st), "matten_radial_pack_cols")
    _lib.check(lib.matten_radial_h_scale(_ptr(w0), _ptr(w1), nb, float(r_start), float(r_end), float(act_cst), _ptr(hs), st),
               "matten_radial_h_scale")
    _lib.check(lib.matten_split_a_tiles(_ptr(w2p), w_pad, _ptr(group_entries), n_ent, _ptr(hs), _ptr(frag), _ptr(inv), st),
               "matten_split_a_tiles")
    return w0p, w1p, w2p, hs, frag, inv


RADIAL_MAX_MID = 3


def _mid(w_mid, name: str):
    if not isinstance(w_mid, torch.Tensor) or w_mid.dim() != 3 or tuple(w_mid.shape[1:]) != (32, 32):
        raise ValueError(f"{name}: expected [n_mid, 32, 32]")
    n_mid = w_mid.shape[0]
    if n_mid > RADIAL_MAX_MID:
        raise ValueError(f"{name}: at most {RADIAL_MAX_MID} middle layers (invariant_layers <= {RADIAL_MAX_MID + 1})")
    return (_need(w_mid, torch.float32, name) if n_mid else None), n_mid


def radial_mlp_deep(geom_sorted, n_basis: int, r_start: float, r_end: float, w0p, w_mid, w2p,
                    out_dtype=torch.float32) -> torch.Tensor:
    lib = _lib.load()
    geom_sorted = _need(geom_sorted, torch.float32, "geom_sorted")
    w0p, w2p = _need(w0p, torch.float32, "w0p"), _need(w2p, torch.float32, "w2p")
    w_mid, n_mid = _mid(w_mid, "w_mid")
    E = geom_sorted.shape[0]
    nb_pad, hidden = w0p.shape
    w_pad = w2p.shape[1]
    if out_dtype not in (torch.float32, torch.bfloat16):
        raise TypeError("radial_mlp: out_dtype must be fp32 or bf16")
    out = torch.empty(E, w_pad, dtype=out_dtype, device=geom_sorted.device)
    with _timed(f"radial_mlp/w_pad={w_pad}"):
        rc = lib.matten_radial_mlp_deep(_ptr(geom_sorted), E, n_basis, r_start, r_end, _ptr(w0p), nb_pad, _ptr(w_mid), n_mid,
                                        _ptr(w2p), hidden, w_pad, 1.0, _ptr(out), int(out_dtype == torch.bfloat16), _stream())
    _lib.check(rc, "matten_radial_mlp_deep")
    return out


def radial_pack_deep(w0, w_mid, w2, scales):
    lib = _lib.load()
    w0, w2 = _need(w0, torch.float32, "layer0.weight"), _need(w2, torch.float32, "last layer weight")
    w_mid, n_mid = _mid(w_mid, "middle layer weights")
    nb, h = w0.shape
    W = w2.shape[1]
    nb_pad, w_pad = (nb + 3) // 4 * 4, (W + 15) // 16 * 16
    dev = w0.device
    w0p = torch.empty(nb_pad, h, dtype=torch.float32, device=dev)
    wmp = torch.empty(n_mid, h, h, dtype=torch.float32, device=dev)
    w2p = torch.empty(h, w_pad, dtype=torch.float32, device=dev)
    _lib.check(lib.matten_radial_pack_deep(_ptr(w0), _ptr(w_mid), n_mid, _ptr(w2), nb, nb_pad, W, w_pad, float(scales[0]),
                                           float(scales[1]), float(scales[2]), _ptr(w0p), _ptr(wmp) if n_mid else None,
                                           _ptr(w2p), _stream()), "matten_radial_pack_deep")
    return w0p, wmp, w2p


def radial_h_scale_deep(w0, w_mid, r_start: float, r_end: float, act_cst: float) -> torch.Tensor:
    lib = _lib.load()
    w0 = _need(w0, torch.float32, "layer0.weight")
    w_mid, n_mid = _mid(w_mid, "middle layer weights")
    hs = torch.empty(2, dtype=torch.float32, device=w0.device)
    _lib.check(lib.matten_radial_h_scale_deep(_ptr(w0), _ptr(w_mid), n_mid, w0.shape[0], float(r_start), float(r_end),
                                              float(act_cst), _ptr(hs), _stream()), "matten_radial_h_scale_deep")
    return hs


def fused_operands_deep(w0, w_mid, w2, scales, cols, group_entries, n_tiles: int, r_start: float, r_end: float,
                        act_cst: float):
    lib = _lib.load()
    w0, w2 = _need(w0, torch.float32, "layer0.weight"), _need(w2, torch.float32, "last layer weight")
    w_mid, n_mid = _mid(w_mid, "middle layer weights")
    cols = _need(cols, torch.int64, "fused_cols")
    group_entries = _need(group_entries, torch.int32, "group_entries")
    nb, h = w0.shape
    W, n_cols = w2.shape[1], cols.numel()
    nb_pad, w_pad = (nb + 3) // 4 * 4, (n_cols + 15) // 16 * 16 + 16
    dev = w0.device
    w0p = torch.empty(nb_pad, h, dtype=torch.float32, device=dev)
    wmp = torch.empty(n_mid, h, h, dtype=torch.float32, device=dev)
    w2p = torch.empty(h, w_pad, dtype=torch.float32, device=dev)
    hs = torch.empty(2, dtype=torch.float32, device=dev)
    n_ent = group_entries.shape[0]
    frag = torch.empty(n_tiles, 64, 16, dtype=torch.float16, device=dev)
    inv = torch.empty(n_ent, dtype=torch.float32, device=dev)
    st = _stream()
    _lib.check(lib.matten_radial_pack_cols_deep(_ptr(w0), _ptr(w_mid), n_mid, _ptr(w2), nb, nb_pad, W, _ptr(cols), n_cols,
                                                w_pad, float(scales[0]), float(scales[1]), float(scales[2]), _ptr(w0p),
                                                _ptr(wmp) if n_mid else None, _ptr(w2p), st), "matten_radial_pack_cols_deep")
    _lib.check(lib.matten_radial_h_scale_deep(_ptr(w0), _ptr(w_mid), n_mid, nb, float(r_start), float(r_end), float(act_cst),
                                              _ptr(hs), st), "matten_radial_h_scale_deep")
    _lib.check(lib.matten_split_a_tiles(_ptr(w2p), w_pad, _ptr(group_entries), n_ent, _ptr(hs), _ptr(frag), _ptr(inv), st),
               "matten_split_a_tiles")
    return w0p, wmp, w2p, hs, frag, inv


def radial_mlp_bwd_deep(geom_sorted, n_basis: int, r_start: float, r_end: float, w0p, w_mid, w2p, w_cols: int, dw,
                        scales=(1.0, 1.0, 1.0)):
    lib = _lib.load()
    geom_sorted = _need(geom_sorted, torch.float32, "geom_sorted")
    w0p, w2p = _need(w0p, torch.float32, "w0p"), _need(w2p, torch.float32, "w2p")
    w_mid, n_mid = _mid(w_mid, "w_mid")
    if dw.dtype not in (torch.float32, torch.bfloat16):
        raise TypeError("dw must be fp32 or bf16")
    dw = _need(dw, dw.dtype, "dw")
    E = geom_sorted.shape[0]
    nb_pad, hidden = w0p.shape
    w_pad = w2p.shape[1]
    dev = geom_sorted.device
    small_len = nb_pad * hidden + n_mid * hidden * hidden
    if E == 0:
        return w0p.new_zeros(nb_pad, hidden), w0p.new_zeros(n_mid, hidden, hidden), w2p.new_zeros(hidden, w_pad)
    n_small, n_rng = lib.matten_radial_mlp_bwd_small_slices(E), lib.matten_radial_mlp_bwd_w2_ranges_deep(E, w_pad, n_mid)
    h2 = torch.empty(E, hidden, dtype=torch.float32, device=dev)
    part_small = torch.empty(max(n_small, 1), small_len, dtype=torch.float32, device=dev)
    part_w2 = torch.empty(max(n_rng, 1), hidden, w_pad, dtype=torch.float32, device=dev)
    small = torch.empty(small_len, dtype=torch.float32, device=dev)
    d2 = torch.empty(hidden, w_pad, dtype=torch.float32, device=dev)
    with _timed(f"radial_mlp_bwd/w_pad={w_pad}"):
        rc = lib.matten_radial_mlp_bwd_deep(_ptr(geom_sorted), E, n_basis, r_start, r_end, _ptr(w0p), nb_pad, _ptr(w_mid),
                                            n_mid, _ptr(w2p), hidden, w_pad, int(w_cols), _ptr(dw), dw.shape[1],
                                            int(dw.dtype == torch.bfloat16), _ptr(h2), _ptr(part_small), _ptr(part_w2),
                                            float(scales[0]), float(scales[1]), float(scales[2]), _ptr(small), _ptr(d2),
                                            _stream())
    _lib.check(rc, "matten_radial_mlp_bwd_deep")
    return small[: nb_pad * hidden].reshape(nb_pad, hidden), small[nb_pad * hidden:].reshape(n_mid, hidden, hidden), d2


def gather_scale(src, idx, scale, scale_by_source: bool = False, perm2=None):
    lib = _lib.load()
    src = _need(src, torch.float32, "src")
    idx = _need(idx, torch.int64, "idx")
    scale = _need(scale, torch.float32, "scale")
    out = torch.empty(idx.shape, dtype=torch.float32, device=src.device)
    out2 = None
    if perm2 is not None:
        perm2 = _need(perm2, torch.int64, "perm2")
        out2 = torch.empty(idx.shape, dtype=torch.float32, device=src.device)
    _lib.check(lib.matten_gather_scale(_ptr(src), _ptr(idx), _ptr(scale), idx.numel(), scale.numel(), int(scale_by_source),
                                       _ptr(out), _ptr(perm2), _ptr(out2), _stream()), "matten_gather_scale")
    return out if perm2 is None else (out, out2)


def radial_mlp_bwd(geom_sorted, n_basis: int, r_start: float, r_end: float, w0p, w1p, w2p, w_cols: int, dw,
                   scales=(1.0, 1.0, 1.0)):
    lib = _lib.load()
    geom_sorted = _need(geom_sorted, torch.float32, "geom_sorted")
    w0p, w1p, w2p = (_need(w, torch.float32, n) for w, n in ((w0p, "w0p"), (w1p, "w1p"), (w2p, "w2p")))
    if dw.dtype not in (torch.float32, torch.bfloat16):
        raise TypeError("dw must be fp32 or bf16")
    dw = _need(dw, dw.dtype, "dw")
    E = geom_sorted.shape[0]
    nb_pad, hidden = w0p.shape
    w_pad = w2p.shape[1]
    dev = geom_sorted.device
    n_small, n_rng = lib.matten_radial_mlp_bwd_small_slices(E), lib.matten_radial_mlp_bwd_w2_ranges(E, w_pad)
    h2 = torch.empty(E, hidden, dtype=torch.float32, device=dev)
    part_small = torch.empty(max(n_small, 1), nb_pad * hidden + hidden * hidden, dtype=torch.float32, device=dev)
    part_w2 = torch.empty(max(n_rng, 1), hidden, w_pad, dtype=torch.float32, device=dev)
    if E == 0:
        return w0p.new_zeros(nb_pad, hidden), w1p.new_zeros(hidden, hidden), w2p.new_zeros(hidden, w_pad)
    small = torch.empty(nb_pad * hidden + hidden * hidden, dtype=torch.float32, device=dev)
    d2 = torch.empty(hidden, w_pad, dtype=torch.float32, device=dev)
    with _timed(f"radial_mlp_bwd/w_pad={w_pad}"):
        rc = lib.matten_radial_mlp_bwd(_ptr(geom_sorted), E, n_basis, r_start, r_end, _ptr(w0p), nb_pad, _ptr(w1p),
                                       _ptr(w2p), hidden, w_pad, int(w_cols), _ptr(dw), dw.shape[1],
                                       int(dw.dtype == torch.bfloat16), _ptr(h2), _ptr(part_small), _ptr(part_w2),
                                       float(scales[0]), float(scales[1]), float(scales[2]), _ptr(small), _ptr(d2),
                                       _stream())
    _lib.check(rc, "matten_radial_mlp_bwd")
    return small[: nb_pad * hidden].reshape(nb_pad, hidden), small[nb_pad * hidden:].reshape(hidden, hidden), d2


def tp_paths(x, w_edge, sh_sorted, rowptr, src_sorted, entries, unit_start, units_per_tile: int, d_mid: int,
             avg_num_neighbors: float, num_neigh=None) -> torch.Tensor:
    lib = _lib.load()
    from .plan import TP_TILE_NODES

    if lib.matten_tp_tile_nodes() != TP_TILE_NODES:
        raise _lib.MattenHipError("plan.TP_TILE_NODES does not match the library's node tile")
    x = _need(x, torch.float32, "node_features")
    w_edge = _edge_dtype(w_edge, "w_edge")
    sh_sorted = _need(sh_sorted, torch.float32, "sh_sorted")
    N, d_in = rowptr.shape[0] - 1, x.shape[1]
    if num_neigh is not None:
        num_neigh = _need(num_neigh, torch.float32, "num_neigh")
    agg = torch.empty(N, d_mid, dtype=torch.float32, device=x.device)
    with _timed(f"tp_scatter/d_mid={d_mid}"):
        rc = lib.matten_tp_paths(_ptr(x), d_in, _ptr(w_edge), w_edge.shape[1], _ptr(sh_sorted), sh_sorted.shape[1],
                                 _ptr(rowptr), _ptr(src_sorted), N, _ptr(entries), _ptr(unit_start),
                                 entries.shape[0], units_per_tile, d_mid, float(avg_num_neighbors or 0.0),
                                 _ptr(num_neigh), _ptr(agg), int(w_edge.dtype == torch.bfloat16), _stream())
    _lib.check(rc, "matten_tp_paths")
    return agg


def split_hidden(h2p: torch.Tensor) -> torch.Tensor:
    tiny = 2.0 ** -14
    hi = torch.where(h2p.abs() < tiny, torch.zeros_like(h2p), h2p.half().float())
    lo = (h2p - hi) * 2048.0
    lo = torch.where(lo.abs() < tiny, torch.zeros_like(lo), lo)
    return torch.stack([hi.half(), lo.half()], dim=1).contiguous()


def radial_hidden(geom_sorted, n_basis: int, r_start: float, r_end: float, w0p, w1p, h_scale=None) -> torch.Tensor:
    lib = _lib.load()
    geom_sorted = _need(geom_sorted, torch.float32, "geom_sorted")
    w0p, w1p = _need(w0p, torch.float32, "w0p"), _need(w1p, torch.float32, "w1p")
    E = geom_sorted.shape[0]
    h2p = torch.empty(E, 2, 32, dtype=torch.float16, device=geom_sorted.device)
    with _timed("radial_hidden"):
        if h_scale is not None:
            h_scale = _need(h_scale, torch.float32, "h_scale")
        rc = lib.matten_radial_hidden(_ptr(geom_sorted), E, n_basis, r_start, r_end, _ptr(w0p), w0p.shape[0],
                                      _ptr(w1p), w0p.shape[1], _ptr(h2p), _ptr(h_scale), _stream())
    _lib.check(rc, "matten_radial_hidden")
    return h2p


def radial_hidden_multi(geom_sorted, n_basis: int, r_start: float, r_end: float, w0ps, w1ps, h_scales=None):
    import ctypes

    lib = _lib.load()
    geom_sorted = _need(geom_sorted, torch.float32, "geom_sorted")
    w0ps = [_need(w, torch.float32, "w0p") for w in w0ps]
    w1ps = [_need(w, torch.float32, "w1p") for w in w1ps]
    L, E = len(w0ps), geom_sorted.shape[0]
    if not 1 <= L <= 8 or len(w1ps) != L or any(w.shape != w0ps[0].shape for w in w0ps):
        raise ValueError("radial_hidden_multi: 1..8 layers with equal basis / hidden sizes")
    out = [torch.empty(E, 2, 32, dtype=torch.float16, device=geom_sorted.device) for _ in range(L)]
    arr = lambda ts: (ctypes.c_void_p * L)(*[t.data_ptr() for t in ts])
    if h_scales is not None:
        h_scales = [_need(h, torch.float32, "h_scale") for h in h_scales]
        if len(h_scales) != L:
            raise ValueError("one h_scale per layer")
    with _timed("radial_hidden_multi"):
        rc = lib.matten_radial_hidden_multi(_ptr(geom_sorted), E, n_basis, r_start, r_end, arr(w0ps), w0ps[0].shape[0],
                                            arr(w1ps), w0ps[0].shape[1], arr(out),
                                            arr(h_scales) if h_scales is not None else None, L, _stream())
    _lib.check(rc, "matten_radial_hidden_multi")
    return out


def radial_hidden_deep(geom_sorted, n_basis: int, r_start: float, r_end: float, w0p, w_mid, h_scale=None) -> torch.Tensor:
    lib = _lib.load()
    geom_sorted = _need(geom_sorted, torch.float32, "geom_sorted")
    w0p = _need(w0p, torch.float32, "w0p")
    w_mid, n_mid = _mid(w_mid, "w_mid")
    E = geom_sorted.shape[0]
    h2p = torch.empty(E, 2, 32, dtype=torch.float16, device=geom_sorted.device)
    with _timed("radial_hidden"):
        if h_scale is not None:
            h_scale = _need(h_scale, torch.float32, "h_scale")
        rc = lib.matten_radial_hidden_deep(_ptr(geom_sorted), E, n_basis, r_start, r_end, _ptr(w0p), w0p.shape[0],
                                           _ptr(w_mid), n_mid, w0p.shape[1], _ptr(h2p), _ptr(h_scale), _stream())
    _lib.check(rc, "matten_radial_hidden_deep")
    return h2p


def radial_hidden_multi_deep(geom_sorted, n_basis: int, r_start: float, r_end: float, w0ps, w_mids, h_scales=None):
    import ctypes

    lib = _lib.load()
    geom_sorted = _need(geom_sorted, torch.float32, "geom_sorted")
    w0ps = [_need(w, torch.float32, "w0p") for w in w0ps]
    mids = [_mid(w, "w_mid") for w in w_mids]
    L, E = len(w0ps), geom_sorted.shape[0]
    if not 1 <= L <= 8 or len(mids) != L or any(w.shape != w0ps[0].shape for w in w0ps) or \
            any(m[1] != mids[0][1] for m in mids):
        raise ValueError("radial_hidden_multi_deep: 1..8 layers with equal basis / hidden sizes and depth")
    n_mid = mids[0][1]
    out = [torch.empty(E, 2, 32, dtype=torch.float16, device=geom_sorted.device) for _ in range(L)]
    arr = lambda ts: (ctypes.c_void_p * L)(*[t.data_ptr() for t in ts])
    if h_scales is not None:
        h_scales = [_need(h, torch.float32, "h_scale") for h in h_scales]
        if len(h_scales) != L:
            raise ValueError("one h_scale per layer")
    with _timed("radial_hidden_multi"):
        rc = lib.matten_radial_hidden_multi_deep(_ptr(geom_sorted), E, n_basis, r_start, r_end, arr(w0ps), w0ps[0].shape[0],
                                                 arr([m[0] for m in mids]) if n_mid else None, n_mid, w0ps[0].shape[1],
                                                 arr(out), arr(h_scales) if h_scales is not None else None, L, _stream())
    _lib.check(rc, "matten_radial_hidden_multi_deep")
    return out


def split_a_tiles(w2p: torch.Tensor, group_entries) -> Tuple[torch.Tensor, torch.Tensor]:
    dev = w2p.device
    g = torch.arange(4, device=dev)[:, None]
    kk = torch.arange(8, device=dev)[None, :]
    k_idx = 16 * (kk >> 2) + 4 * g + (kk & 3)
    tiny = 2.0 ** -14
    tiles, inv = [], []
    for row in np.asarray(group_entries).reshape(-1, 32):
        w_base, n_mt = int(row[5]), int(row[7])
        if int(row[0]) < 0 or n_mt == 0:
            inv.append(torch.ones((), device=dev))
            continue
        A = w2p[k_idx][:, :, w_base:w_base + 16 * n_mt]
        A = A.reshape(4, 8, n_mt, 16).permute(2, 0, 3, 1)
        amax = A.abs().max()
        e = torch.where(amax > 0, (torch.frexp(amax)[1] - 1).clamp(-100, 100), torch.full_like(amax, 13, dtype=torch.int32))
        scale = torch.ldexp(torch.ones_like(amax), 13 - e)
        inv.append(torch.ldexp(torch.ones_like(amax), e - 13))
        v = A * scale
        hi = torch.where(v.abs() < tiny, torch.zeros_like(v), v.half().float())
        lo = (v - hi) * 2048.0
        lo = torch.where(lo.abs() < tiny, torch.zeros_like(lo), lo)
        tiles.append(torch.cat([hi.half(), lo.half()], dim=-1).reshape(n_mt, 64, 16))
    return torch.cat(tiles).contiguous(), torch.stack(inv).float().contiguous()


_GROUPS_CHECKED = False


def tp_fused(x, h2p, w2p, sh_sorted, rowptr, src_sorted, entries, unit_map, units_per_tile: int,
             lds_floats_per_wave: int, d_mid: int, avg_num_neighbors: float, num_neigh=None,
             a_split=None) -> torch.Tensor:
    lib = _lib.load()
    from .plan import TP_TILE_NODES

    if lib.matten_tp_tile_nodes() != TP_TILE_NODES:
        raise _lib.MattenHipError("plan.TP_TILE_NODES does not match the library's node tile")
    from .plan import TP_MAX_COLS, TP_MAX_COLS_L0, TP_MAX_COLS_L1
    if (lib.matten_tp_max_cols() != TP_MAX_COLS or lib.matten_tp_max_cols_l0() != TP_MAX_COLS_L0
            or lib.matten_tp_max_cols_l1() != TP_MAX_COLS_L1):
        raise _lib.MattenHipError("plan.TP_MAX_COLS does not match the library's entry width (-DTPF_MAX_COLS)")
    global _GROUPS_CHECKED
    from .plan import tp_groups_hash
    if not _GROUPS_CHECKED and lib.matten_tp_groups_hash() != tp_groups_hash():
        raise _lib.MattenHipError("the library's coupling code (cg_gen.h) was generated for other coupling groups than plan.TP_GROUPS "
                                  "(MATTEN_TP_GROUPS / an interrupted tools/*.sh A/B build?): make -C matten_amd/csrc clean all")
    _GROUPS_CHECKED = True
    x = _need_rows(x, torch.float32, "node_features")
    h2p = _need(h2p, torch.float16, "h2s")
    if h2p.dim() != 3 or h2p.shape[1:] != (2, 32):
        raise ValueError(f"h2s must be [E,2,32] fp16 (ops.split_hidden / ops.radial_hidden), got {tuple(h2p.shape)}")
    w2p = _need(w2p, torch.float32, "w2p")
    sh_sorted = _need(sh_sorted, torch.float32, "sh_sorted")
    N, d_in = rowptr.shape[0] - 1, x.stride(0)
    if num_neigh is not None:
        num_neigh = _need(num_neigh, torch.float32, "num_neigh")
    if a_split is not None:
        a_split = (_need(a_split[0], torch.float16, "a_split"), _need(a_split[1], torch.float32, "a_scale_inv"))
        if a_split[1].numel() != entries.shape[0]:
            raise ValueError("a_scale_inv needs one value per group entry")
    if unit_map.numel() != units_per_tile:
        raise ValueError(f"unit_map has {unit_map.numel()} units, expected {units_per_tile} (plan.fused_unit_map)")
    agg = torch.empty(N, d_mid, dtype=torch.float32, device=x.device)
    with _timed(f"tp_scatter/d_mid={d_mid}/d_in={x.shape[1]}"):
        rc = lib.matten_tp_fused(_ptr(x), d_in, _ptr(h2p), _ptr(w2p), w2p.shape[1], _ptr(sh_sorted),
                                 sh_sorted.shape[1], _ptr(rowptr), _ptr(src_sorted), N, _ptr(entries),
                                 _ptr(unit_map), entries.shape[0], units_per_tile, lds_floats_per_wave, d_mid,
                                 float(avg_num_neighbors or 0.0), _ptr(num_neigh),
                                 _ptr(a_split[0]) if a_split is not None else None,
                                 _ptr(a_split[1]) if a_split is not None else None, _ptr(agg), _stream())
    _lib.check(rc, "matten_tp_fused")
    return agg


def agg_linear(agg, species_order, wtab, io_table, blocks, d_out: int, add=None) -> torch.Tensor:
    lib = _lib.load()
    from .plan import AGG_BLOCK, AGG_MAX_MT
    if lib.matten_agg_linear_block_chunks() != AGG_BLOCK or lib.matten_agg_linear_max_mt() != AGG_MAX_MT:
        raise _lib.MattenHipError("plan.AGG_BLOCK / AGG_MAX_MT do not match the library (-DAL_BLK_CHUNKS)")
    agg = _need(agg, torch.float32, "agg")
    wtab = _need(wtab, torch.float32, "A fragments")
    n_rows, ld = agg.shape
    order, seg = species_order if species_order is not None else (None, None)
    n_species = wtab.shape[0] if wtab.dim() == 2 else 1
    if add is not None:
        add = _need_rows(add, torch.float32, "add")
    out = torch.empty(n_rows, d_out, dtype=torch.float32, device=agg.device)
    with _timed(f"agg_linear/ld={ld}"):
        rc = lib.matten_agg_linear(_ptr(agg), ld, _ptr(order), _ptr(seg), n_species, _ptr(wtab), wtab.shape[-1],
                                   _ptr(io_table), io_table.shape[0], _ptr(blocks), blocks.shape[0], _ptr(add),
                                   add.stride(0) if add is not None else d_out, d_out, n_rows, _ptr(out), _stream())
    _lib.check(rc, "matten_agg_linear")
    return out


def agg_linear_gate(agg, species_order, wtab, io_table, blocks, d_out: int, cmeta, act_cst, d_act: int, add=None,
                    bn_scale=None, bn_shift=None) -> torch.Tensor:
    lib = _lib.load()
    from .plan import AGG_BLOCK, AGG_GATE_SETS, AGG_MAX_MT
    if (lib.matten_agg_linear_block_chunks() != AGG_BLOCK or lib.matten_agg_linear_max_mt() != AGG_MAX_MT
            or lib.matten_agg_linear_gate_sets() != AGG_GATE_SETS):
        raise _lib.MattenHipError("plan.AGG_BLOCK / AGG_MAX_MT / AGG_GATE_SETS do not match the library")
    agg = _need(agg, torch.float32, "agg")
    wtab = _need(wtab, torch.float32, "A fragments")
    n_rows, ld = agg.shape
    order, seg = species_order if species_order is not None else (None, None)
    n_species = wtab.shape[0] if wtab.dim() == 2 else 1
    if add is not None:
        add = _need_rows(add, torch.float32, "add")
    if cmeta.shape != (d_out, 4):
        raise ValueError("cmeta must be [d_out, 4]")
    if bn_scale is not None:
        bn_scale, bn_shift = _need(bn_scale, torch.float32, "bn_scale"), _need(bn_shift, torch.float32, "bn_shift")
        if bn_scale.numel() != d_act or bn_shift.numel() != d_act:
            raise ValueError("bn_scale / bn_shift must have one value per activated column")
    out = torch.empty(n_rows, d_act, dtype=torch.float32, device=agg.device)
    with _timed(f"agg_linear/ld={ld}"):
        rc = lib.matten_agg_linear_gate(_ptr(agg), ld, _ptr(order), _ptr(seg), n_species, _ptr(wtab), wtab.shape[-1],
                                        _ptr(io_table), io_table.shape[0], _ptr(blocks), blocks.shape[0], _ptr(add),
                                        add.stride(0) if add is not None else d_out, d_out, n_rows, _ptr(cmeta),
                                        _ptr(act_cst), _ptr(bn_scale), _ptr(bn_shift), d_act, _ptr(out), _stream())
    _lib.check(rc, "matten_agg_linear_gate")
    return out


_SL_ROWS_LDS_BYTES = 52 * 1024


def species_linear(x, species_order, wp, w_stride: int, item_tables, d_out: int, add=None,
                   fully_covered: bool = True, variant: Optional[str] = None) -> torch.Tensor:
    lib = _lib.load()
    x = _need(x, torch.float32, "x")
    from . import selfcheck
    selfcheck.check_species_linear(x.device)
    wp = _need(wp, torch.float32, "packed weights")
    n_rows, d_in = x.shape
    order, seg = species_order if species_order is not None else (None, None)
    n_species = wp.shape[0] if wp.dim() == 2 else 1
    cur_add = add
    if cur_add is not None:
        cur_add = _need_rows(cur_add, torch.float32, "add")
    if fully_covered:
        out = torch.empty(n_rows, d_out, dtype=torch.float32, device=x.device)
    else:
        out = cur_add.clone() if cur_add is not None else torch.zeros(n_rows, d_out, dtype=torch.float32, device=x.device)
    rows_fits = len(item_tables) == 1 and 4 * (16 * (d_in | 1) + w_stride + 8 * item_tables[0].shape[0] + 4) <= _SL_ROWS_LDS_BYTES
    rows_variant = rows_fits and os.environ.get("MATTEN_SL_ROWS", "1") != "0"
    if variant is not None:
        rows_variant = rows_fits and variant == "rows"
    for items in item_tables:
        fn = lib.matten_species_linear_rows if rows_variant else lib.matten_species_linear
        _lib.check(
            fn(_ptr(x), d_in, _ptr(order), _ptr(seg), n_species, _ptr(wp), w_stride,
                                      _ptr(items), items.shape[0], d_out, _ptr(cur_add),
                                      cur_add.stride(0) if cur_add is not None else d_out, n_rows, _ptr(out), _stream()),
            "matten_species_linear",
        )
        cur_add = out
    return out


def gate_bn(x, meta, act_cst, running_mean=None, running_var=None, bn_weight=None, bn_bias=None, eps: float = 1e-5):
    lib = _lib.load()
    x = _need(x, torch.float32, "x")
    n_rows, d_in = x.shape
    d_out = meta.shape[0]
    out = torch.empty(n_rows, d_out, dtype=torch.float32, device=x.device)
    _lib.check(
        lib.matten_gate_bn(_ptr(x), d_in, _ptr(meta), d_out, _ptr(act_cst), _ptr(running_mean), _ptr(running_var),
                           _ptr(bn_weight), _ptr(bn_bias), eps, n_rows, _ptr(out), _stream()),
        "matten_gate_bn",
    )
    return out


def segment_reduce(x, ptr, mean: bool) -> torch.Tensor:
    lib = _lib.load()
    x = _need(x, torch.float32, "x")
    ptr = _need(ptr, torch.int64, "ptr")
    B = ptr.shape[0] - 1
    out = torch.empty(B, x.shape[1], dtype=torch.float32, device=x.device)
    _lib.check(lib.matten_segment_reduce(_ptr(x), x.shape[1], _ptr(ptr), B, int(mean), _ptr(out), _stream()),
               "matten_segment_reduce")
    return out


def segment_minmax(x, ptr, take_max: bool, want_arg: bool = False):
    lib = _lib.load()
    x = _need(x, torch.float32, "x")
    ptr = _need(ptr, torch.int64, "ptr")
    B = ptr.shape[0] - 1
    out = torch.empty(B, x.shape[1], dtype=torch.float32, device=x.device)
    arg = torch.empty(B, x.shape[1], dtype=torch.int64, device=x.device) if want_arg else None
    _lib.check(lib.matten_segment_minmax(_ptr(x), x.shape[1], _ptr(ptr), B, int(take_max), _ptr(out), _ptr(arg), _stream()),
               "matten_segment_minmax")
    return (out, arg) if want_arg else out


def segment_minmax_bwd(dy, arg, n_rows: int) -> torch.Tensor:
    lib = _lib.load()
    dy = _need(dy, torch.float32, "dy")
    dx = torch.zeros(n_rows, dy.shape[1], dtype=torch.float32, device=dy.device)
    _lib.check(lib.matten_segment_minmax_bwd(_ptr(dy), dy.shape[1], _ptr(arg), dy.shape[0], _ptr(dx), _stream()),
               "matten_segment_minmax_bwd")
    return dx


def dense_rows(x, q) -> torch.Tensor:
    lib = _lib.load()
    x = _need(x, torch.float32, "x")
    q = _need(q, torch.float32, "q")
    out = torch.empty(x.shape[0], q.shape[1], dtype=torch.float32, device=x.device)
    _lib.check(lib.matten_dense_rows(_ptr(x), x.shape[1], _ptr(q), q.shape[1], x.shape[0], _ptr(out), _stream()),
               "matten_dense_rows")
    return out


def tp_backward(x, w_edge, sh_sorted, src_sorted, dst_sorted, col_meta, nnz_ijk, nnz_c, g_agg,
                avg_num_neighbors: float, num_neigh=None, in_groups=None):
    lib = _lib.load()
    x = _need(x, torch.float32, "x")
    w_edge = _edge_dtype(w_edge, "w_edge")
    g_agg = _need(g_agg, torch.float32, "grad agg")
    N, d_in = x.shape
    E = w_edge.shape[0]
    W = col_meta.shape[0]
    dx = torch.zeros(N, d_in, dtype=torch.float32, device=x.device)
    dw = torch.empty(E, w_edge.shape[1], dtype=w_edge.dtype, device=x.device)
    if num_neigh is not None:
        num_neigh = _need(num_neigh, torch.float32, "num_neigh")
    with _timed(f"tp_backward/d_mid={g_agg.shape[1]}/d_in={d_in}"):
        rc = lib.matten_tp_backward(_ptr(x), d_in, _ptr(w_edge), w_edge.shape[1], _ptr(sh_sorted), sh_sorted.shape[1],
                                    _ptr(src_sorted), _ptr(dst_sorted), _ptr(col_meta), W, _ptr(nnz_ijk), _ptr(nnz_c),
                                    _ptr(g_agg), g_agg.shape[1], float(avg_num_neighbors or 0.0), _ptr(num_neigh), E,
                                    _ptr(dx), _ptr(dw), dw.shape[1], _ptr(in_groups[0]) if in_groups else None,
                                    _ptr(in_groups[1]) if in_groups else None,
                                    in_groups[0].shape[0] - 1 if in_groups else 0,
                                    int(w_edge.dtype == torch.bfloat16), _stream())
    _lib.check(rc, "matten_tp_backward")
    return dx, dw


def split_a_tiles_dev(w2p, entries, n_tiles: int, h_scale=None):
    lib = _lib.load()
    w2p = _need(w2p, torch.float32, "w2p")
    entries = _need(entries, torch.int32, "entries")
    frag = torch.empty(n_tiles, 64, 16, dtype=torch.float16, device=w2p.device)
    inv = torch.empty(entries.shape[0], dtype=torch.float32, device=w2p.device)
    _lib.check(lib.matten_split_a_tiles(_ptr(w2p), w2p.shape[1], _ptr(entries), entries.shape[0], _ptr(h_scale), _ptr(frag),
                                        _ptr(inv), _stream()), "matten_split_a_tiles")
    return frag, inv


WFREE_MAX_MUL = 256


def tp_backward_lit(x, w_edge, sh_sorted, src_sorted, dst_sorted, blocks, paths, sum_lanes: int, g_agg,
                    avg_num_neighbors: float, num_neigh=None, out_csr=None, blocks_cover_input: bool = True, wfree=None,
                    dw_shape=None, lds_floats: int = 4096, max_l: int = 4, max_mul: int = 256):
    lib = _lib.load()
    x = _need(x, torch.float32, "x")
    g_agg = _need(g_agg, torch.float32, "grad agg")
    N, d_in = x.shape
    if wfree is not None:
        if w_edge is not None or dw_shape is None:
            raise ValueError("wfree: pass w_edge=None and dw_shape=((E, ld), dtype)")
        h2s, frag, w_inv = (_need(t, dt, n) for t, dt, n in zip(wfree, (torch.float16, torch.float16, torch.float32),
                                                                ("h2s", "frag", "w_inv")))
        (E, dw_ld), dw_dtype = dw_shape
        if h2s.shape != (E, 2, 32) or w_inv.numel() != paths.shape[0]:
            raise ValueError("wfree: h2s must be [E, 2, 32] and w_inv hold one value per path")
    else:
        w_edge = _edge_dtype(w_edge, "w_edge")
        E, dw_ld, dw_dtype = w_edge.shape[0], w_edge.shape[1], w_edge.dtype
    if out_csr is not None:
        out_ptr, out_perm = (_need(t, torch.int32, n) for t, n in zip(out_csr, ("out_ptr", "out_perm")))
        dx = torch.empty(N, d_in, dtype=torch.float32, device=x.device)
        dx_edges = (torch.empty if blocks_cover_input else torch.zeros)(E, d_in, dtype=torch.float32, device=x.device)
    else:
        out_ptr = out_perm = dx_edges = None
        dx = torch.zeros(N, d_in, dtype=torch.float32, device=x.device)
    dw = torch.empty(E, dw_ld, dtype=dw_dtype, device=x.device)
    if num_neigh is not None:
        num_neigh = _need(num_neigh, torch.float32, "num_neigh")
    if wfree is not None:
        with _timed(f"tp_backward/d_mid={g_agg.shape[1]}/d_in={d_in}"):
            rc = lib.matten_tp_backward_lit_wfree(_ptr(x), d_in, _ptr(h2s), _ptr(frag), _ptr(w_inv), _ptr(sh_sorted),
                                                  sh_sorted.shape[1], _ptr(src_sorted), _ptr(dst_sorted), _ptr(blocks),
                                                  blocks.shape[0], int(sum_lanes), _ptr(paths), paths.shape[0], _ptr(g_agg),
                                                  g_agg.shape[1], float(avg_num_neighbors or 0.0), _ptr(num_neigh), E, _ptr(dx),
                                                  _ptr(dw), dw_ld, int(dw_dtype == torch.bfloat16), N, _ptr(out_ptr),
                                                  _ptr(out_perm), _ptr(dx_edges), int(lds_floats), int(max_l), int(max_mul),
                                                  _stream())
        _lib.check(rc, "matten_tp_backward_lit_wfree")
        return dx, dw
    with _timed(f"tp_backward/d_mid={g_agg.shape[1]}/d_in={d_in}"):
        rc = lib.matten_tp_backward_lit(_ptr(x), d_in, _ptr(w_edge), w_edge.shape[1], _ptr(sh_sorted), sh_sorted.shape[1],
                                        _ptr(src_sorted), _ptr(dst_sorted), _ptr(blocks), blocks.shape[0], int(sum_lanes),
                                        _ptr(paths), paths.shape[0], _ptr(g_agg), g_agg.shape[1],
                                        float(avg_num_neighbors or 0.0), _ptr(num_neigh), E, _ptr(dx), _ptr(dw),
                                        dw.shape[1], int(w_edge.dtype == torch.bfloat16), N, _ptr(out_ptr), _ptr(out_perm),
                                        _ptr(dx_edges), int(max_l), _stream())
    _lib.check(rc, "matten_tp_backward_lit")
    return dx, dw


def species_linear_wgrad(x, dy, species_order, n_species: int, seg_tables, w_stride: int) -> torch.Tensor:
    lib = _lib.load()
    x = _need(x, torch.float32, "x")
    dy = _need(dy, torch.float32, "dy")
    order, seg = species_order if species_order is not None else (None, None)
    n_scratch = lib.matten_species_linear_wgrad_scratch_floats(x.shape[0], n_species, w_stride)
    dwp = torch.empty(n_species, w_stride, dtype=torch.float32, device=x.device)
    partial = torch.empty(n_scratch, dtype=torch.float32, device=x.device) if n_scratch > 0 else None
    for segs in seg_tables:
        _lib.check(
            lib.matten_species_linear_wgrad(_ptr(x), x.shape[1], _ptr(dy), dy.shape[1], _ptr(order), _ptr(seg),
                                            n_species, x.shape[0], _ptr(segs), segs.shape[0], w_stride, _ptr(dwp),
                                            _ptr(partial), _stream()),
            "matten_species_linear_wgrad",
        )
    return dwp


def gate_bwd(x, meta, act_cst, dy) -> torch.Tensor:
    lib = _lib.load()
    x = _need(x, torch.float32, "x")
    dy = _need(dy, torch.float32, "dy")
    dx = torch.empty_like(x)
    _lib.check(lib.matten_gate_bwd(_ptr(x), x.shape[1], _ptr(meta), meta.shape[0], _ptr(act_cst), _ptr(dy), x.shape[0],
                                   _ptr(dx), _stream()), "matten_gate_bwd")
    return dx


def _bn_scratch(lib, x):
    n = lib.matten_bn_scratch_floats(x.shape[0], x.shape[1])
    return torch.empty(n, dtype=torch.float32, device=x.device) if n > 0 else None


def bn_train_fwd(x, col2chan, chan, weight, bias, eps: float, running_mean=None, running_var=None, momentum: float = 0.0):
    lib = _lib.load()
    x = _need(x, torch.float32, "x")
    C = chan.shape[0]
    mean = torch.empty(C, dtype=torch.float32, device=x.device)
    nu = torch.empty(C, dtype=torch.float32, device=x.device)
    y = torch.empty_like(x)
    if running_var is not None:
        running_mean = _need(running_mean, torch.float32, "running_mean")
        running_var = _need(running_var, torch.float32, "running_var")
    scratch = _bn_scratch(lib, x)
    _lib.check(lib.matten_bn_train_fwd(_ptr(x), x.shape[1], x.shape[0], _ptr(col2chan), _ptr(chan), C, _ptr(weight),
                                       _ptr(bias), eps, _ptr(mean), _ptr(nu), _ptr(y), _ptr(running_mean),
                                       _ptr(running_var), float(momentum), _ptr(scratch), _stream()),
               "matten_bn_train_fwd")
    if running_var is not None:
        bump_weights_epoch()
    return y, mean, nu


def norm_act(x, chan, act: int, epsilon: float = 1e-8, running_mean=None, running_var=None, bn_weight=None, bn_bias=None,
             bn_eps: float = 1e-5) -> torch.Tensor:
    lib = _lib.load()
    x = _need(x, torch.float32, "x")
    y = torch.empty_like(x)
    _lib.check(lib.matten_norm_act(_ptr(x), x.shape[1], x.shape[0], _ptr(chan), chan.shape[0], int(act), float(epsilon),
                                   _ptr(running_mean), _ptr(running_var), _ptr(bn_weight), _ptr(bn_bias), float(bn_eps),
                                   _ptr(y), _stream()), "matten_norm_act")
    return y


def norm_act_bwd(x, dy, chan, act: int, epsilon: float = 1e-8) -> torch.Tensor:
    lib = _lib.load()
    dy = _need(dy, torch.float32, "dy")
    dx = torch.empty_like(x)
    _lib.check(lib.matten_norm_act_bwd(_ptr(x), _ptr(dy), x.shape[1], x.shape[0], _ptr(chan), chan.shape[0], int(act),
                                       float(epsilon), _ptr(dx), _stream()), "matten_norm_act_bwd")
    return dx


def _bn_eval_bwd_outputs(lib, x, n_cols: int, n_chan: int, n_bias: int, param_grads: bool):
    dx = torch.empty_like(x)
    if not param_grads:
        return dx, None, None, None
    dweight = torch.empty(n_chan, dtype=torch.float32, device=x.device)
    dbias = torch.empty(n_bias, dtype=torch.float32, device=x.device)
    scratch = torch.empty(lib.matten_bn_eval_bwd_scratch_floats(x.shape[0], n_cols), dtype=torch.float32, device=x.device)
    return dx, dweight, dbias, scratch


def gate_bn_eval_bwd(x, meta, act_cst, bn_chan, running_mean, running_var, bn_weight, eps: float, dy, n_bias: int,
                     param_grads: bool = True):
    lib = _lib.load()
    x = _need(x, torch.float32, "x")
    dy = _need(dy, torch.float32, "dy")
    if x.shape[0] == 0:
        z = (lambda n: torch.zeros(n, dtype=torch.float32, device=x.device)) if param_grads else (lambda n: None)
        return torch.empty_like(x), z(bn_chan.shape[0]), z(n_bias)
    d_out, C = meta.shape[0], bn_chan.shape[0]
    dx, dweight, dbias, scratch = _bn_eval_bwd_outputs(lib, x, d_out, C, n_bias, param_grads)
    _lib.check(lib.matten_gate_bn_eval_bwd(_ptr(x), x.shape[1], _ptr(meta), d_out, _ptr(act_cst), _ptr(bn_chan), C,
                                           _ptr(running_mean), _ptr(running_var), _ptr(bn_weight), float(eps), _ptr(dy),
                                           x.shape[0], _ptr(dx), _ptr(dweight), _ptr(dbias), _ptr(scratch), _stream()),
               "matten_gate_bn_eval_bwd")
    return dx, dweight, dbias


def norm_act_bn_eval_bwd(x, dy, chan, act: int, epsilon: float, running_mean, running_var, bn_weight, bn_eps: float,
                         n_bias: int, param_grads: bool = True):
    lib = _lib.load()
    x = _need(x, torch.float32, "x")
    dy = _need(dy, torch.float32, "dy")
    C = chan.shape[0]
    if x.shape[0] == 0:
        z = (lambda n: torch.zeros(n, dtype=torch.float32, device=x.device)) if param_grads else (lambda n: None)
        return torch.empty_like(x), z(C), z(n_bias)
    dx, dweight, dbias, scratch = _bn_eval_bwd_outputs(lib, x, C, C, n_bias, param_grads)
    _lib.check(lib.matten_norm_act_bn_eval_bwd(_ptr(x), _ptr(dy), x.shape[1], x.shape[0], _ptr(chan), C, int(act),
                                               float(epsilon), _ptr(running_mean), _ptr(running_var), _ptr(bn_weight),
                                               float(bn_eps), _ptr(dx), _ptr(dweight), _ptr(dbias), _ptr(scratch),
                                               _stream()), "matten_norm_act_bn_eval_bwd")
    return dx, dweight, dbias


def instance_norm_fwd(x, seg_ptr, seg_of_row, col2chan, chan, weight, bias, eps: float):
    lib = _lib.load()
    x = _need(x, torch.float32, "x")
    seg_ptr = _need(seg_ptr, torch.int64, "ptr")
    seg_of_row = _need(seg_of_row, torch.int64, "batch")
    C, B = chan.shape[0], seg_ptr.shape[0] - 1
    mean = torch.empty(B, C, dtype=torch.float32, device=x.device)
    nu = torch.empty(B, C, dtype=torch.float32, device=x.device)
    y = torch.empty_like(x)
    _lib.check(lib.matten_instance_norm_fwd(_ptr(x), x.shape[1], x.shape[0], _ptr(seg_ptr), _ptr(seg_of_row), B,
                                            _ptr(col2chan), _ptr(chan), C, _ptr(weight), _ptr(bias), eps, _ptr(mean),
                                            _ptr(nu), _ptr(y), _stream()), "matten_instance_norm_fwd")
    return y, mean, nu


def instance_norm_bwd(x, dy, seg_ptr, seg_of_row, col2chan, chan, mean, nu, weight, eps: float):
    lib = _lib.load()
    dy = _need(dy, torch.float32, "dy")
    B, C = mean.shape
    A = torch.empty(B, C, dtype=torch.float32, device=x.device)
    Bs = torch.empty(B, C, dtype=torch.float32, device=x.device)
    dx = torch.empty_like(x)
    _lib.check(lib.matten_instance_norm_bwd(_ptr(x), _ptr(dy), x.shape[1], x.shape[0], _ptr(seg_ptr), _ptr(seg_of_row), B,
                                            _ptr(col2chan), _ptr(chan), C, _ptr(mean), _ptr(nu), _ptr(weight), eps,
                                            _ptr(A), _ptr(Bs), _ptr(dx), _stream()), "matten_instance_norm_bwd")
    return dx, A, Bs


def bn_train_bwd(x, dy, col2chan, chan, mean, nu, weight, eps: float, n_bias: int):
    lib = _lib.load()
    dy = _need(dy, torch.float32, "dy")
    C = chan.shape[0]
    A = torch.empty(C, dtype=torch.float32, device=x.device)
    B = torch.empty(C, dtype=torch.float32, device=x.device)
    dweight = torch.empty(C, dtype=torch.float32, device=x.device)
    dbias = torch.empty(n_bias, dtype=torch.float32, device=x.device)
    dx = torch.empty_like(x)
    scratch = _bn_scratch(lib, x)
    _lib.check(lib.matten_bn_train_bwd(_ptr(x), _ptr(dy), x.shape[1], x.shape[0], _ptr(col2chan), _ptr(chan), C,
                                       _ptr(mean), _ptr(nu), _ptr(weight), eps, _ptr(A), _ptr(B), _ptr(dx), _ptr(dweight),
                                       _ptr(dbias), _ptr(scratch), _stream()),
               "matten_bn_train_bwd")
    return dx, dweight, dbias


def segment_reduce_bwd(dy, ptr, n_rows: int, mean: bool) -> torch.Tensor:
    lib = _lib.load()
    dy = _need(dy, torch.float32, "dy")
    ptr = _need(ptr, torch.int64, "ptr")
    dx = torch.zeros(n_rows, dy.shape[1], dtype=torch.float32, device=dy.device)
    _lib.check(lib.matten_segment_reduce_bwd(_ptr(dy), dy.shape[1], _ptr(ptr), dy.shape[0], int(mean), _ptr(dx),
                                             _stream()), "matten_segment_reduce_bwd")
    return dx


def graph_prep(pos64, cell64, ptr, r_cut: float):
    lib = _lib.load()
    pos64 = _need(pos64, torch.float64, "pos")
    cell64 = _need(cell64, torch.float64, "cell")
    ptr = _need(ptr, torch.int64, "ptr")
    N, B, dev = pos64.shape[0], ptr.shape[0] - 1, pos64.device
    frac = torch.empty(N, 3, dtype=torch.float64, device=dev)
    bound = torch.empty(B, 3, dtype=torch.float64, device=dev)
    batch = torch.empty(N, dtype=torch.int64, device=dev)
    pos32 = torch.empty(N, 3, dtype=torch.float32, device=dev)
    cell32 = torch.empty(3 * B, 3, dtype=torch.float32, device=dev)
    _lib.check(lib.matten_graph_prep(_ptr(pos64), _ptr(cell64), _ptr(ptr), B, float(r_cut), _ptr(frac), _ptr(bound),
                                     _ptr(batch), _ptr(pos32), _ptr(cell32), _stream()), "matten_graph_prep")
    return frac, bound, batch, pos32, cell32


def neighbor_list(pos64, cell64, ptr, frac, bound, pair_ptr, r_cut: float, max_atoms: int, n_pairs: int, want_csr: bool = True):
    lib = _lib.load()
    pos64 = _need(pos64, torch.float64, "pos")
    cell64 = _need(cell64, torch.float64, "cell")
    ptr = _need(ptr, torch.int64, "ptr")
    frac = _need(frac, torch.float64, "frac")
    bound = _need(bound, torch.float64, "bound")
    pair_ptr = _need(pair_ptr, torch.int64, "pair_ptr")
    B = ptr.shape[0] - 1
    N = pos64.shape[0]
    dev = pos64.device
    counts = torch.empty((2 if want_csr else 1) * n_pairs, dtype=torch.int32, device=dev)
    with _timed("neighbor_count"):
        _lib.check(
            lib.matten_neighbor_count(_ptr(pos64), _ptr(cell64), _ptr(ptr), _ptr(frac), _ptr(bound), _ptr(pair_ptr),
                                      float(r_cut), B, int(max_atoms), _ptr(counts),
                                      counts.data_ptr() + 4 * n_pairs if (want_csr and n_pairs) else None, _stream()),
            "matten_neighbor_count",
        )
    scan = torch.zeros(counts.numel() + 1, dtype=torch.int64, device=dev)
    torch.cumsum(counts, 0, dtype=torch.int64, out=scan[1:])
    offsets = scan[: n_pairs + 1]
    if n_pairs:
        summary = torch.empty(2, dtype=torch.int64, device=dev)
        _lib.check(lib.matten_neighbor_summary(_ptr(offsets), _ptr(pair_ptr), B, _ptr(summary), _stream()),
                   "matten_neighbor_summary")
        E, min_edges = summary.tolist()
    else:
        E, min_edges = 0, 0
    edge_index = torch.empty(2, E, dtype=torch.int64, device=dev)
    shifts = torch.empty(E, 3, dtype=torch.float32, device=dev)
    num_neigh = torch.empty(N, dtype=torch.float32, device=dev)
    csr = offsets_t = None
    if want_csr and n_pairs and E < 2 ** 31:
        offsets_t = scan[n_pairs:]
        csr = (torch.empty(E, dtype=torch.int32, device=dev), torch.empty(N + 1, dtype=torch.int32, device=dev),
               torch.empty(E, dtype=torch.int32, device=dev))
    with _timed("neighbor_fill"):
        _lib.check(
            lib.matten_neighbor_fill(_ptr(pos64), _ptr(cell64), _ptr(ptr), _ptr(frac), _ptr(bound), _ptr(pair_ptr),
                                     float(r_cut), B, int(max_atoms), _ptr(offsets), E, _ptr(edge_index), _ptr(shifts),
                                     _ptr(num_neigh), _ptr(offsets_t), N, _ptr(csr[1]) if csr else None,
                                     _ptr(csr[2]) if csr else None, _ptr(csr[0]) if csr else None, _stream()),
            "matten_neighbor_fill",
        )
    return edge_index, shifts, num_neigh, offsets, int(min_edges), csr
```

Before: 1.271 billion edge-TP/s.

## Fuse CSR scan into count kernel and species histogram into embedding

After: 1.152 billion edge-TP/s. -9.4%, worse.

```diff
diff --git a/include/matten_hip.h b/include/matten_hip.h
--- a/include/matten_hip.h
+++ b/include/matten_hip.h
@@ -24,6 +24,10 @@
 int matten_csr_build(const int64_t* edge_index, int64_t n_edges, int64_t n_nodes, int32_t* perm,
                      int32_t* rowptr, int32_t* src_sorted, void* workspace, size_t workspace_bytes,
                      int32_t* err_flag, matten_stream_t stream);
+int64_t matten_csr_counter_words(int64_t n_nodes);
+int matten_csr_build_zeroed(const int64_t* edge_index, int64_t n_edges, int64_t n_nodes, int32_t* perm,
+                            int32_t* rowptr, int32_t* src_sorted, void* workspace, size_t workspace_bytes,
+                            int32_t* err_flag, int32_t* counters, matten_stream_t stream);
 
 int64_t matten_csr_split_bound(int64_t n_nodes, int64_t n_edges, int64_t max_len);
 int matten_csr_split(const int32_t* rowptr, int64_t n_nodes, int64_t n_edges, int64_t max_len, int32_t* vrowptr,
@@ -32,11 +36,19 @@
 size_t matten_group_workspace_bytes(int64_t n, int64_t n_keys);
 int matten_group_by_key(const int64_t* key, int64_t n, int64_t n_keys, int32_t* order, int32_t* seg,
                         void* workspace, size_t workspace_bytes, int32_t* err_flag, matten_stream_t stream);
+int matten_group_self_scan(int64_t n, int64_t n_keys);
+int matten_group_place(const int64_t* key, int64_t n, int64_t n_keys, const int32_t* run_hist, int32_t* order,
+                       int32_t* seg, int32_t* err_flag, matten_stream_t stream);
 
 int matten_species_embed(const int64_t* atomic_numbers, int64_t n_nodes, const int64_t* z_to_index,
                          int64_t min_z, int64_t max_z, int64_t n_species, const float* weight ,
                          const float* bias , int64_t dim, int64_t* species_index, int32_t* species_i32,
                          float* node_feats, float* node_attrs, int32_t* err_flag, matten_stream_t stream);
+int matten_species_embed_hist(const int64_t* atomic_numbers, int64_t n_nodes, const int64_t* z_to_index,
+                              int64_t min_z, int64_t max_z, int64_t n_species, const float* weight ,
+                              const float* bias , int64_t dim, int64_t* species_index, int32_t* species_i32,
+                              float* node_feats, float* node_attrs, int32_t* err_flag, int32_t* run_hist,
+                              int32_t* zero, int64_t n_zero, matten_stream_t stream);
 
 int matten_edge_geom(const float* pos, const int64_t* edge_index, const float* edge_cell_shift,
                      const float* cell, int64_t n_cells, const int64_t* batch, const int32_t* perm,
diff --git a/matten_amd/_lib.py b/matten_amd/_lib.py
--- a/matten_amd/_lib.py
+++ b/matten_amd/_lib.py
@@ -16,10 +16,16 @@
     "matten_group_workspace_bytes": (c_size_t, [c_int64, c_int64]),
     "matten_csr_counting_max_avg_degree": (c_int, []),
     "matten_csr_build": (c_int, [P, c_int64, c_int64, P, P, P, P, c_size_t, P, P]),
+    "matten_csr_counter_words": (c_int64, [c_int64]),
+    "matten_csr_build_zeroed": (c_int, [P, c_int64, c_int64, P, P, P, P, c_size_t, P, P, P]),
     "matten_csr_split_bound": (c_int64, [c_int64, c_int64, c_int64]),
     "matten_csr_split": (c_int, [P, c_int64, c_int64, c_int64, P, P, P, P, P]),
     "matten_group_by_key": (c_int, [P, c_int64, c_int64, P, P, P, c_size_t, P, P]),
+    "matten_group_self_scan": (c_int, [c_int64, c_int64]),
+    "matten_group_place": (c_int, [P, c_int64, c_int64, P, P, P, P, P]),
     "matten_species_embed": (c_int, [P, c_int64, P, c_int64, c_int64, c_int64, P, P, c_int64, P, P, P, P, P, P]),
+    "matten_species_embed_hist": (c_int, [P, c_int64, P, c_int64, c_int64, c_int64, P, P, c_int64, P, P, P, P, P, P, P,
+                                          c_int64, P]),
     "matten_edge_geom": (c_int, [P, P, P, P, c_int64, P, P, c_int64, c_int64, c_int, c_int, c_float, c_float, P, P, c_int, P, P, P, P, P]),
     "matten_radial_mlp": (c_int, [P, c_int64, c_int, c_float, c_float, P, c_int, P, P, c_int, c_int, c_float, P, c_int, P]),
     "matten_radial_mlp_deep": (c_int, [P, c_int64, c_int, c_float, c_float, P, c_int, P, c_int, P, c_int, c_int, c_float, P, c_int,
diff --git a/matten_amd/csrc/csr.hip b/matten_amd/csrc/csr.hip
--- a/matten_amd/csrc/csr.hip
+++ b/matten_amd/csrc/csr.hip
@@ -47,17 +47,98 @@
     if (i < n) p[i] = 0;
 }
 
-__global__ void csr_count_kernel(const int64_t* __restrict__ edge_index, int64_t E, int64_t N,
-                                 int32_t* __restrict__ deg, int32_t* __restrict__ slot, int32_t* err_flag) {
-    int64_t e = (int64_t)blockIdx.x * blockDim.x + threadIdx.x;
-    if (e >= E) return;
-    int64_t s = edge_index[e];
-    int64_t d = edge_index[E + e];
-    if (s < 0 || s >= N || d < 0 || d >= N) {
-        atomicOr(err_flag, 1);
-        d = d < 0 ? 0 : (d >= N ? N - 1 : d);
-    }
-    slot[e] = atomicAdd(&deg[d], 1);
+constexpr int CSR_HUB_DEGREE = 2048;
+constexpr int CSR_HUB_THREADS = 1024;
+constexpr int CSR_HUB_BLOCKS = 64;
+
+constexpr int CSR_COUNT_THREADS = 1024;
+constexpr int CSR_SCAN_TILE = CSR_COUNT_THREADS * 4;
+constexpr int CSR_SCAN_TILES = 4;
+inline int64_t csr_counter_pad(int64_t N) { return (N + 4) & ~(int64_t)3; }
+inline int64_t csr_counter_words(int64_t N) { return csr_counter_pad(N) + 4; }
+
+__global__ __launch_bounds__(CSR_COUNT_THREADS) void csr_count_kernel(const int64_t* __restrict__ edge_index, int64_t E,
+                                                                      int64_t N, int32_t* counters,
+                                                                      int32_t* __restrict__ slot,
+                                                                      int32_t* __restrict__ rowptr,
+                                                                      int32_t* __restrict__ hubs, int32_t* err_flag) {
+    __shared__ int wave_tot[CSR_SCAN_TILES][CSR_COUNT_THREADS / 64];
+    __shared__ int last_s;
+    const int t = threadIdx.x;
+    const int64_t e = (int64_t)blockIdx.x * blockDim.x + t;
+    if (e < E) {
+        int64_t s = edge_index[e];
+        int64_t d = edge_index[E + e];
+        if (s < 0 || s >= N || d < 0 || d >= N) {
+            atomicOr(err_flag, 1);
+            d = d < 0 ? 0 : (d >= N ? N - 1 : d);
+        }
+        slot[e] = atomicAdd(&counters[d], 1);
+    }
+    const int64_t cw = (N + 4) & ~(int64_t)3;
+    __threadfence();
+    __syncthreads();
+    if (t == 0) last_s = atomicAdd(&counters[cw], 1) == (int)gridDim.x - 1;
+    __syncthreads();
+    if (!last_s) return;
+    __threadfence();
+    const int lane = t & 63, wave = t >> 6;
+    const bool vec_out = (reinterpret_cast<uintptr_t>(rowptr) & 15) == 0;
+    int carry = 0;
+    for (int64_t base = 0; base < cw; base += (int64_t)CSR_SCAN_TILE * CSR_SCAN_TILES) {
+        int4 v[CSR_SCAN_TILES];
+        int incl[CSR_SCAN_TILES], sum[CSR_SCAN_TILES];
+#pragma unroll
+        for (int q = 0; q < CSR_SCAN_TILES; ++q) {
+            const int64_t i = base + (int64_t)q * CSR_SCAN_TILE + 4 * t;
+            v[q] = i < cw ? *reinterpret_cast<const int4*>(counters + i) : make_int4(0, 0, 0, 0);
+        }
+#pragma unroll
+        for (int q = 0; q < CSR_SCAN_TILES; ++q) {
+            if (hubs) {
+                const int64_t i = base + (int64_t)q * CSR_SCAN_TILE + 4 * t;
+                const int dd[4] = {v[q].x, v[q].y, v[q].z, v[q].w};
+#pragma unroll
+                for (int c = 0; c < 4; ++c)
+                    if (dd[c] > CSR_HUB_DEGREE) hubs[atomicAdd(&counters[cw + 1], 1)] = (int32_t)(i + c);
+            }
+            sum[q] = v[q].x + v[q].y + v[q].z + v[q].w;
+            int x = sum[q];
+            for (int off = 1; off < 64; off <<= 1) {
+                const int y = __shfl_up(x, off);
+                if (lane >= off) x += y;
+            }
+            incl[q] = x;
+            if (lane == 63) wave_tot[q][wave] = x;
+        }
+        __syncthreads();
+        int run = carry;
+#pragma unroll
+        for (int q = 0; q < CSR_SCAN_TILES; ++q) {
+            int off = run;
+            for (int w = 0; w < CSR_COUNT_THREADS / 64; ++w) {
+                const int wt = wave_tot[q][w];
+                if (w < wave) off += wt;
+                run += wt;
+            }
+            const int64_t i = base + (int64_t)q * CSR_SCAN_TILE + 4 * t;
+            int4 o;
+            o.x = off + incl[q] - sum[q];
+            o.y = o.x + v[q].x;
+            o.z = o.y + v[q].y;
+            o.w = o.z + v[q].z;
+            if (vec_out && i + 3 <= N) {
+                *reinterpret_cast<int4*>(rowptr + i) = o;
+            } else {
+                if (i <= N) rowptr[i] = o.x;
+                if (i + 1 <= N) rowptr[i + 1] = o.y;
+                if (i + 2 <= N) rowptr[i + 2] = o.z;
+                if (i + 3 <= N) rowptr[i + 3] = o.w;
+            }
+        }
+        carry = run;
+        __syncthreads();
+    }
 }
 
 __global__ void csr_place_kernel(const int64_t* __restrict__ edge_index, int64_t E, int64_t N,
@@ -70,21 +151,48 @@
     ids[rowptr[d] + slot[e]] = (int32_t)e;
 }
 
-constexpr int CSR_HUB_DEGREE = 2048;
-constexpr int CSR_HUB_THREADS = 1024;
-constexpr int CSR_HUB_BLOCKS = 64;
-
-__global__ void csr_rank_kernel(const int64_t* __restrict__ edge_index, const int32_t* __restrict__ rowptr,
-                                const int32_t* __restrict__ ids, int64_t E, int64_t N, int32_t* __restrict__ perm,
-                                int32_t* __restrict__ src_sorted, int32_t* __restrict__ hubs) {
+__global__ __launch_bounds__(CSR_HUB_THREADS) void csr_rank_kernel(const int64_t* __restrict__ edge_index,
+                                                                   const int32_t* __restrict__ rowptr, int32_t* ids,
+                                                                   int64_t E, int64_t N, int32_t* __restrict__ perm,
+                                                                   int32_t* __restrict__ src_sorted,
+                                                                   const int32_t* __restrict__ hubs,
+                                                                   const int32_t* __restrict__ n_hubs_p,
+                                                                   int rank_blocks) {
+    if ((int)blockIdx.x >= rank_blocks) {
+        const int n_hubs = *n_hubs_p;
+        for (int h = blockIdx.x - rank_blocks; h < n_hubs; h += gridDim.x - rank_blocks) {
+            const int node = hubs[h];
+            const int beg = rowptr[node], d = rowptr[node + 1] - beg;
+            int32_t* a = ids + beg;
+            for (int64_t k = 2; (k >> 1) < d; k <<= 1) {
+                for (int64_t j = k >> 1; j > 0; j >>= 1) {
+                    const int64_t m = (j == (k >> 1)) ? k - 1 : j;
+                    for (int64_t i = threadIdx.x; i < d; i += CSR_HUB_THREADS) {
+                        const int64_t l = i ^ m;
+                        if (l > i && l < d) {
+                            const int32_t x = a[i], y = a[l];
+                            if (y < x) a[i] = y, a[l] = x;
+                        }
+                    }
+                    __syncthreads();
+                }
+            }
+            for (int64_t i = threadIdx.x; i < d; i += CSR_HUB_THREADS) {
+                const int32_t id = a[i];
+                perm[beg + i] = id;
+                int64_t s = edge_index[id];
+                s = s < 0 ? 0 : (s >= N ? N - 1 : s);
+                src_sorted[beg + i] = (int32_t)s;
+            }
+            __syncthreads();
+        }
+        return;
+    }
     const int64_t node = ((int64_t)blockIdx.x * blockDim.x + threadIdx.x) >> 4;
     if (node >= N) return;
     const int sub = threadIdx.x & 15;
     const int beg = rowptr[node], d = rowptr[node + 1] - beg;
-    if (d > CSR_HUB_DEGREE) {
-        if (sub == 0) hubs[atomicAdd(&hubs[N], 1)] = (int32_t)node;
-        return;
-    }
+    if (d > CSR_HUB_DEGREE) return;
     for (int i = sub; i < d; i += 16) {
         const int id = ids[beg + i];
         int rank = 0;
@@ -101,40 +209,6 @@
         int64_t s = edge_index[id];
         s = s < 0 ? 0 : (s >= N ? N - 1 : s);
         src_sorted[beg + rank] = (int32_t)s;
-    }
-}
-
-__global__ __launch_bounds__(CSR_HUB_THREADS) void csr_hub_kernel(const int64_t* __restrict__ edge_index,
-                                                                  const int32_t* __restrict__ rowptr, int32_t* ids,
-                                                                  int64_t N, int32_t* __restrict__ perm,
-                                                                  int32_t* __restrict__ src_sorted,
-                                                                  const int32_t* __restrict__ hubs) {
-    const int n_hubs = hubs[N];
-    for (int h = blockIdx.x; h < n_hubs; h += gridDim.x) {
-        const int node = hubs[h];
-        const int beg = rowptr[node], d = rowptr[node + 1] - beg;
-        int32_t* a = ids + beg;
-        for (int64_t k = 2; (k >> 1) < d; k <<= 1) {
-            for (int64_t j = k >> 1; j > 0; j >>= 1) {
-                const int64_t m = (j == (k >> 1)) ? k - 1 : j;
-                for (int64_t i = threadIdx.x; i < d; i += CSR_HUB_THREADS) {
-                    const int64_t l = i ^ m;
-                    if (l > i && l < d) {
-                        const int32_t x = a[i], y = a[l];
-                        if (y < x) a[i] = y, a[l] = x;
-                    }
-                }
-                __syncthreads();
-            }
-        }
-        for (int64_t i = threadIdx.x; i < d; i += CSR_HUB_THREADS) {
-            const int32_t id = a[i];
-            perm[beg + i] = id;
-            int64_t s = edge_index[id];
-            s = s < 0 ? 0 : (s >= N ? N - 1 : s);
-            src_sorted[beg + i] = (int32_t)s;
-        }
-        __syncthreads();
     }
 }
 
@@ -202,6 +276,71 @@
     if (k >= 0) order[offs[(int64_t)k * n_runs + run] + rank] = (int32_t)i;
 }
 
+constexpr int64_t GROUP_SELF_SCAN_MAX = 16384;
+
+__global__ __launch_bounds__(GROUP_WAVES * 64) void group_place_scan_kernel(const int64_t* __restrict__ key, int64_t n,
+                                                                            int n_keys, int n_runs,
+                                                                            const int32_t* __restrict__ cnt,
+                                                                            int32_t* __restrict__ order,
+                                                                            int32_t* __restrict__ seg, int32_t* err_flag) {
+    __shared__ int tot[GROUP_COUNTING_MAX_KEYS], pre[GROUP_COUNTING_MAX_KEYS], sc[GROUP_COUNTING_MAX_KEYS];
+    const int t = threadIdx.x, lane = t & 63, wv = t >> 6;
+    const int r0 = blockIdx.x * GROUP_WAVES;
+    tot[t] = 0;
+    pre[t] = 0;
+    __syncthreads();
+    const int table = n_keys * n_runs;
+    for (int i0 = t; i0 < table; i0 += 8 * GROUP_WAVES * 64) {
+        int v[8];
+#pragma unroll
+        for (int q = 0; q < 8; ++q) {
+            const int i = i0 + q * GROUP_WAVES * 64;
+            v[q] = i < table ? cnt[i] : 0;
+        }
+#pragma unroll
+        for (int q = 0; q < 8; ++q) {
+            if (v[q]) {
+                const int i = i0 + q * GROUP_WAVES * 64;
+                const int k = i / n_runs;
+                atomicAdd(&tot[k], v[q]);
+                if (i - k * n_runs < r0) atomicAdd(&pre[k], v[q]);
+            }
+        }
+    }
+    __syncthreads();
+    const int mine = t < n_keys ? tot[t] : 0;
+    sc[t] = mine;
+    __syncthreads();
+    for (int off = 1; off < GROUP_WAVES * 64; off <<= 1) {
+        const int v = t >= off ? sc[t - off] : 0;
+        __syncthreads();
+        sc[t] += v;
+        __syncthreads();
+    }
+    const int first = sc[t] - mine;
+    pre[t] += first;
+    if (blockIdx.x == 0) {
+        if (t < n_keys) seg[t] = first;
+        if (t == 0) seg[n_keys] = (int32_t)n;
+    }
+    __syncthreads();
+    const int64_t i = (int64_t)blockIdx.x * blockDim.x + t;
+    const int k = group_key_of(key, i, n, n_keys, err_flag);
+    unsigned long long todo = __ballot(k >= 0);
+    int rank = 0;
+    while (todo) {
+        const int kf = __shfl(k, __ffsll((long long)todo) - 1);
+        const unsigned long long m = __ballot(k == kf);
+        if (k == kf) rank = __popcll(m & ((1ull << lane) - 1ull));
+        todo &= ~m;
+    }
+    if (k >= 0) {
+        int off = pre[k];
+        for (int w = 0; w < wv; ++w) off += cnt[k * n_runs + r0 + w];
+        order[off + rank] = (int32_t)i;
+    }
+}
+
 inline size_t align256(size_t x) { return (x + 255) & ~(size_t)255; }
 
 inline int key_bits(int64_t N) {
@@ -268,8 +407,8 @@
     (void)rocprim::radix_sort_pairs(nullptr, tmp, p, p, p, p, (size_t)(E > 0 ? E : 1), 0, key_bits(N), 0, false);
     size_t scan_tmp = 0;
     (void)rocprim::exclusive_scan(nullptr, scan_tmp, p, p, 0, (size_t)(N + 1), rocprim::plus<int32_t>());
-    return 3 * align256((size_t)(E > 0 ? E : 1) * sizeof(int32_t)) + align256(tmp) + align256((size_t)(N + 1) * sizeof(int32_t)) +
-           align256(scan_tmp) + 256;
+    return 3 * align256((size_t)(E > 0 ? E : 1) * sizeof(int32_t)) + align256(tmp) +
+           align256((size_t)csr_counter_words(N) * sizeof(int32_t)) + align256(scan_tmp) + 256;
 }
 
 extern "C" size_t matten_group_workspace_bytes(int64_t n, int64_t n_keys) {
@@ -290,12 +429,15 @@
 
 extern "C" int matten_csr_counting_max_avg_degree(void) { return (int)CSR_COUNTING_MAX_AVG_DEGREE; }
 
-extern "C" int matten_csr_build(const int64_t* edge_index, int64_t E, int64_t N, int32_t* perm, int32_t* rowptr,
-                                int32_t* src_sorted, void* workspace, size_t workspace_bytes, int32_t* err_flag,
-                                matten_stream_t stream_) {
+extern "C" int64_t matten_csr_counter_words(int64_t n_nodes) { return n_nodes < 0 ? 0 : csr_counter_words(n_nodes); }
+
+extern "C" int matten_csr_build_zeroed(const int64_t* edge_index, int64_t E, int64_t N, int32_t* perm, int32_t* rowptr,
+                                       int32_t* src_sorted, void* workspace, size_t workspace_bytes, int32_t* err_flag,
+                                       int32_t* counters, matten_stream_t stream_) {
     hipStream_t stream = (hipStream_t)stream_;
     if (E < 0 || N < 0 || N >= ((int64_t)1 << 31) || E >= ((int64_t)1 << 31)) return MATTEN_EINVAL;
     if (!rowptr || !err_flag) return MATTEN_EINVAL;
+    if (counters && (reinterpret_cast<uintptr_t>(counters) & 15)) return MATTEN_EINVAL;
     if (E == 0) {
         zero_i32_kernel<<<(unsigned)matten_cdiv(N + 1, 256), 256, 0, stream>>>(rowptr, N + 1);
         MATTEN_LAUNCH_CHECK();
@@ -317,28 +459,24 @@
     if (N > 0 && E <= CSR_COUNTING_MAX_AVG_DEGREE * N) {
         int32_t* ids = (int32_t*)ws;
         int32_t* slot = (int32_t*)(ws + seg);
-        int32_t* deg = (int32_t*)(ws + 2 * seg);
-        const size_t deg_bytes = align256((size_t)(N + 1) * sizeof(int32_t));
-        void* scan_tmp = ws + 2 * seg + deg_bytes;
-        size_t scan_bytes = workspace_bytes - 2 * seg - deg_bytes;
-        zero_i32_kernel<<<(unsigned)matten_cdiv(N + 1, T), T, 0, stream>>>(deg, N + 1);
-        MATTEN_LAUNCH_CHECK();
-        csr_count_kernel<<<(unsigned)matten_cdiv(E, T), T, 0, stream>>>(edge_index, E, N, deg, slot, err_flag);
-        MATTEN_LAUNCH_CHECK();
-        if (rocprim::exclusive_scan(scan_tmp, scan_bytes, deg, rowptr, 0, (size_t)(N + 1), rocprim::plus<int32_t>(),
-                                    stream) != hipSuccess)
-            return MATTEN_ELAUNCH;
+        int32_t* hubs = E > CSR_HUB_DEGREE ? (int32_t*)(ws + 2 * seg) : nullptr;
+        const int64_t cw = csr_counter_pad(N);
+        if (!counters) {
+            counters = (int32_t*)(ws + 3 * seg);
+            zero_i32_kernel<<<(unsigned)matten_cdiv(cw + 4, T), T, 0, stream>>>(counters, cw + 4);
+            MATTEN_LAUNCH_CHECK();
+        }
+        csr_count_kernel<<<(unsigned)matten_cdiv(E, CSR_COUNT_THREADS), CSR_COUNT_THREADS, 0, stream>>>(
+            edge_index, E, N, counters, slot, rowptr, hubs, err_flag);
+        MATTEN_LAUNCH_CHECK();
         csr_place_kernel<<<(unsigned)matten_cdiv(E, T), T, 0, stream>>>(edge_index, E, N, rowptr, slot, ids);
         MATTEN_LAUNCH_CHECK();
-        csr_rank_kernel<<<(unsigned)matten_cdiv(N * 16, T), T, 0, stream>>>(edge_index, rowptr, ids, E, N, perm,
-                                                                           src_sorted, deg);
-        MATTEN_LAUNCH_CHECK();
-        if (E > CSR_HUB_DEGREE) {
-            const int64_t max_hubs = E / CSR_HUB_DEGREE;
-            csr_hub_kernel<<<(unsigned)(max_hubs < CSR_HUB_BLOCKS ? max_hubs : CSR_HUB_BLOCKS), CSR_HUB_THREADS, 0,
-                             stream>>>(edge_index, rowptr, ids, N, perm, src_sorted, deg);
-            MATTEN_LAUNCH_CHECK();
-        }
+        const int64_t rank_blocks = matten_cdiv(N * 16, CSR_HUB_THREADS);
+        const int64_t max_hubs = E / CSR_HUB_DEGREE;
+        const int64_t hub_blocks = hubs ? (max_hubs < CSR_HUB_BLOCKS ? max_hubs : CSR_HUB_BLOCKS) : 0;
+        csr_rank_kernel<<<(unsigned)(rank_blocks + hub_blocks), CSR_HUB_THREADS, 0, stream>>>(
+            edge_index, rowptr, ids, E, N, perm, src_sorted, hubs, counters + cw + 1, (int)rank_blocks);
+        MATTEN_LAUNCH_CHECK();
         return MATTEN_OK;
     }
     csr_keys_kernel<<<(unsigned)matten_cdiv(E, T), T, 0, stream>>>(edge_index, E, N, keys_in, vals_in, err_flag);
@@ -351,6 +489,13 @@
     csr_src_kernel<<<(unsigned)matten_cdiv(E, T), T, 0, stream>>>(edge_index, perm, E, N, src_sorted);
     MATTEN_LAUNCH_CHECK();
     return MATTEN_OK;
+}
+
+extern "C" int matten_csr_build(const int64_t* edge_index, int64_t E, int64_t N, int32_t* perm, int32_t* rowptr,
+                                int32_t* src_sorted, void* workspace, size_t workspace_bytes, int32_t* err_flag,
+                                matten_stream_t stream_) {
+    return matten_csr_build_zeroed(edge_index, E, N, perm, rowptr, src_sorted, workspace, workspace_bytes, err_flag,
+                                   nullptr, stream_);
 }
 
 extern "C" int matten_group_by_key(const int64_t* key, int64_t n, int64_t n_keys, int32_t* order, int32_t* seg,
@@ -378,6 +523,12 @@
         group_hist_kernel<<<(unsigned)matten_cdiv(n_runs, GROUP_WAVES), TB, 0, stream>>>(key, n, n_keys, n_runs, cnt,
                                                                                         err_flag);
         MATTEN_LAUNCH_CHECK();
+        if ((int64_t)table <= GROUP_SELF_SCAN_MAX) {
+            group_place_scan_kernel<<<(unsigned)matten_cdiv(n, TB), TB, 0, stream>>>(key, n, (int)n_keys, (int)n_runs, cnt,
+                                                                                    order, seg, err_flag);
+            MATTEN_LAUNCH_CHECK();
+            return MATTEN_OK;
+        }
         if (rocprim::exclusive_scan(scan_tmp, scan_bytes, cnt, offs, 0, table, rocprim::plus<int32_t>(), stream) !=
             hipSuccess)
             return MATTEN_ELAUNCH;
@@ -400,6 +551,21 @@
                                   stream, false) != hipSuccess)
         return MATTEN_ELAUNCH;
     csr_rowptr_kernel<<<(unsigned)matten_cdiv(n_keys + 1, T), T, 0, stream>>>(keys_out, n, n_keys, seg);
+    MATTEN_LAUNCH_CHECK();
+    return MATTEN_OK;
+}
+
+extern "C" int matten_group_self_scan(int64_t n, int64_t n_keys) {
+    return n > 0 && n_keys > 0 && n_keys <= GROUP_COUNTING_MAX_KEYS && n_keys * ((n + 63) / 64) <= GROUP_SELF_SCAN_MAX;
+}
+
+extern "C" int matten_group_place(const int64_t* key, int64_t n, int64_t n_keys, const int32_t* run_hist, int32_t* order,
+                                  int32_t* seg, int32_t* err_flag, matten_stream_t stream_) {
+    if (!matten_group_self_scan(n, n_keys) || n >= ((int64_t)1 << 31)) return MATTEN_EINVAL;
+    if (!key || !run_hist || !order || !seg || !err_flag) return MATTEN_EINVAL;
+    const int TB = GROUP_WAVES * 64;
+    group_place_scan_kernel<<<(unsigned)matten_cdiv(n, TB), TB, 0, (hipStream_t)stream_>>>(
+        key, n, (int)n_keys, (int)((n + 63) / 64), run_hist, order, seg, err_flag);
     MATTEN_LAUNCH_CHECK();
     return MATTEN_OK;
 }
diff --git a/matten_amd/csrc/edge.hip b/matten_amd/csrc/edge.hip
--- a/matten_amd/csrc/edge.hip
+++ b/matten_amd/csrc/edge.hip
@@ -85,34 +85,78 @@
     }
 }
 
-__global__ void species_embed_kernel(const int64_t* __restrict__ Z, int64_t N, const int64_t* __restrict__ lut,
-                                     int64_t min_z, int64_t max_z, int64_t S, const float* __restrict__ W,
-                                     const float* __restrict__ b, int64_t dim, int64_t* __restrict__ species_index,
-                                     int32_t* __restrict__ species_i32, float* __restrict__ feats,
-                                     float* __restrict__ attrs, int32_t* err_flag) {
-    int64_t n = (int64_t)blockIdx.x * blockDim.y + threadIdx.y;
-    if (n >= N) return;
-    int64_t z = Z[n];
-    int64_t idx = -1;
-    if (z < min_z || z > max_z) {
-        if (threadIdx.x == 0) atomicOr(err_flag, 2);
-    } else {
-        idx = lut[z - min_z];
-        if (idx < 0 || idx >= S) {
-            if (threadIdx.x == 0) atomicOr(err_flag, 4);
-            idx = -1;
+constexpr int EMBED_RUN = 64;
+constexpr int EMBED_THREADS = 256;
+constexpr int EMBED_HIST_MAX_SPECIES = 256;
+
+__global__ __launch_bounds__(EMBED_THREADS) void species_embed_kernel(
+    const int64_t* __restrict__ Z, int64_t N, const int64_t* __restrict__ lut, int64_t min_z, int64_t max_z, int64_t S,
+    const float* __restrict__ W, const float* __restrict__ b, int dim, int64_t* __restrict__ species_index,
+    int32_t* __restrict__ species_i32, float* __restrict__ feats, float* __restrict__ attrs, int32_t* err_flag,
+    int32_t* __restrict__ run_hist, int64_t n_runs, int32_t* __restrict__ zero, int64_t n_zero) {
+    __shared__ int idx_s[EMBED_RUN];
+    __shared__ int h[EMBED_HIST_MAX_SPECIES];
+    const int t = threadIdx.x;
+    for (int64_t i = (int64_t)blockIdx.x * EMBED_THREADS + t; i < n_zero; i += (int64_t)gridDim.x * EMBED_THREADS)
+        zero[i] = 0;
+    if (run_hist) h[t] = 0;
+    __syncthreads();
+    const int64_t n0 = (int64_t)blockIdx.x * EMBED_RUN;
+    if (t < EMBED_RUN) {
+        const int64_t n = n0 + t;
+        int64_t idx = -1;
+        if (n < N) {
+            const int64_t z = Z[n];
+            if (z < min_z || z > max_z) {
+                atomicOr(err_flag, 2);
+            } else {
+                idx = lut[z - min_z];
+                if (idx < 0 || idx >= S) {
+                    atomicOr(err_flag, 4);
+                    idx = -1;
+                }
+            }
+            if (species_index) species_index[n] = idx;
+            if (species_i32) species_i32[n] = (int32_t)(idx < 0 ? 0 : idx);
+            if (run_hist) atomicAdd(&h[idx < 0 ? 0 : idx], 1);
         }
+        idx_s[t] = (int)idx;
     }
-    if (threadIdx.x == 0) {
-        if (species_index) species_index[n] = idx;
-        if (species_i32) species_i32[n] = (int32_t)(idx < 0 ? 0 : idx);
+    __syncthreads();
+    const int rows = (int)(N - n0 < EMBED_RUN ? N - n0 : EMBED_RUN);
+    for (int j = t; j < rows * dim; j += EMBED_THREADS) {
+        const int r = j / dim, d = j - r * dim;
+        const int idx = idx_s[r];
+        feats[n0 * dim + j] = W[(int64_t)d * S + (idx < 0 ? 0 : idx)] + b[d];
     }
-    int64_t s = idx < 0 ? 0 : idx;
-    for (int64_t d = threadIdx.x; d < dim; d += blockDim.x) feats[n * dim + d] = W[d * S + s] + b[d];
     if (attrs)
-        for (int64_t c = threadIdx.x; c < S; c += blockDim.x) attrs[n * S + c] = (c == idx) ? 1.0f : 0.0f;
+        for (int64_t j = t; j < rows * S; j += EMBED_THREADS) {
+            const int r = (int)(j / S);
+            attrs[n0 * S + j] = ((j - r * S) == idx_s[r]) ? 1.0f : 0.0f;
+        }
+    if (run_hist)
+        for (int k = t; k < S; k += EMBED_THREADS) run_hist[(int64_t)k * n_runs + blockIdx.x] = h[k];
 }
 
+}
+
+extern "C" int matten_species_embed_hist(const int64_t* atomic_numbers, int64_t n_nodes, const int64_t* z_to_index,
+                                         int64_t min_z, int64_t max_z, int64_t n_species, const float* weight,
+                                         const float* bias, int64_t dim, int64_t* species_index, int32_t* species_i32,
+                                         float* node_feats, float* node_attrs, int32_t* err_flag, int32_t* run_hist,
+                                         int32_t* zero, int64_t n_zero, matten_stream_t stream_) {
+    hipStream_t stream = (hipStream_t)stream_;
+    if (n_nodes < 0 || dim <= 0 || n_species <= 0 || n_zero < 0 || dim >= ((int64_t)1 << 20)) return MATTEN_EINVAL;
+    if (run_hist && n_species > EMBED_HIST_MAX_SPECIES) return MATTEN_EINVAL;
+    if (n_zero > 0 && (!zero || n_nodes == 0)) return MATTEN_EINVAL;
+    if (n_nodes == 0) return MATTEN_OK;
+    if (!atomic_numbers || !z_to_index || !weight || !bias || !node_feats || !err_flag) return MATTEN_EINVAL;
+    const int64_t n_runs = matten_cdiv(n_nodes, EMBED_RUN);
+    species_embed_kernel<<<(unsigned)n_runs, EMBED_THREADS, 0, stream>>>(
+        atomic_numbers, n_nodes, z_to_index, min_z, max_z, n_species, weight, bias, (int)dim, species_index, species_i32,
+        node_feats, node_attrs, err_flag, run_hist, n_runs, zero, n_zero);
+    MATTEN_LAUNCH_CHECK();
+    return MATTEN_OK;
 }
 
 extern "C" int matten_species_embed(const int64_t* atomic_numbers, int64_t n_nodes, const int64_t* z_to_index,
@@ -120,16 +164,9 @@
                                     const float* bias, int64_t dim, int64_t* species_index, int32_t* species_i32,
                                     float* node_feats, float* node_attrs, int32_t* err_flag,
                                     matten_stream_t stream_) {
-    hipStream_t stream = (hipStream_t)stream_;
-    if (n_nodes < 0 || dim <= 0 || n_species <= 0) return MATTEN_EINVAL;
-    if (n_nodes == 0) return MATTEN_OK;
-    if (!atomic_numbers || !z_to_index || !weight || !bias || !node_feats || !err_flag) return MATTEN_EINVAL;
-    dim3 block(16, 16);
-    species_embed_kernel<<<(unsigned)matten_cdiv(n_nodes, 16), block, 0, stream>>>(
-        atomic_numbers, n_nodes, z_to_index, min_z, max_z, n_species, weight, bias, dim, species_index, species_i32,
-        node_feats, node_attrs, err_flag);
-    MATTEN_LAUNCH_CHECK();
-    return MATTEN_OK;
+    return matten_species_embed_hist(atomic_numbers, n_nodes, z_to_index, min_z, max_z, n_species, weight, bias, dim,
+                                     species_index, species_i32, node_feats, node_attrs, err_flag, nullptr, nullptr, 0,
+                                     stream_);
 }
 
 extern "C" int matten_edge_geom(const float* pos, const int64_t* edge_index, const float* edge_cell_shift,
diff --git a/matten_amd/nn/_nequip.py b/matten_amd/nn/_nequip.py
--- a/matten_amd/nn/_nequip.py
+++ b/matten_amd/nn/_nequip.py
@@ -14,10 +14,10 @@
     return data
 
 
-def ensure_graph(data: DataKey.Type, err=None) -> DataKey.Type:
+def ensure_graph(data: DataKey.Type, err=None, counters=None) -> DataKey.Type:
     if DataKey.AMD_ROWPTR not in data:
         n_nodes = data[DataKey.POSITIONS].shape[0]
-        perm, rowptr, src, err = ops.csr_build(data[DataKey.EDGE_INDEX], n_nodes, err=err)
+        perm, rowptr, src, err = ops.csr_build(data[DataKey.EDGE_INDEX], n_nodes, err=err, counters=counters)
         data[DataKey.AMD_PERM], data[DataKey.AMD_ROWPTR], data[DataKey.AMD_SRC] = perm, rowptr, src
         data["_amd_csr_err"] = err
     return data
diff --git a/matten_amd/nn/embedding.py b/matten_amd/nn/embedding.py
--- a/matten_amd/nn/embedding.py
+++ b/matten_amd/nn/embedding.py
@@ -120,17 +120,26 @@
         else:
             raise ValueError("Nothing in `data` to encode. Need either species_index or atomic_numbers")
         flags_dev = torch.zeros(3, dtype=torch.int32, device=Z.device)
+        n = Z.shape[0]
+        run_hist = ops.group_run_hist(n, S, Z.device)
+        counters = None
+        if n > 0 and DataKey.EDGE_INDEX in data and DataKey.AMD_ROWPTR not in data:
+            counters = ops.csr_counters(data[DataKey.EDGE_INDEX].shape[1], data[DataKey.POSITIONS].shape[0], Z.device)
         sidx, s32, feats, attrs, _ = ops.species_embed(
-            Z, lut, lo, hi, S, self.linear.weight, self.linear.bias, want_attrs=self.materialize, err=flags_dev[0:1]
+            Z, lut, lo, hi, S, self.linear.weight, self.linear.bias, want_attrs=self.materialize, err=flags_dev[0:1],
+            run_hist=run_hist, zero=counters,
         )
         if DataKey.EDGE_INDEX in data:
             from ._nequip import ensure_graph
 
             built_here = DataKey.AMD_ROWPTR not in data
-            csr_err = ensure_graph(data, err=flags_dev[1:2]).get("_amd_csr_err")
+            csr_err = ensure_graph(data, err=flags_dev[1:2], counters=counters).get("_amd_csr_err")
             if not built_here and csr_err is not None:
                 flags_dev[1:2] = csr_err
-        order, seg, _ = ops.group_by_key(sidx, S, err=flags_dev[2:3])
+        if run_hist is not None:
+            order, seg, _ = ops.group_place(sidx, S, run_hist, err=flags_dev[2:3])
+        else:
+            order, seg, _ = ops.group_by_key(sidx, S, err=flags_dev[2:3])
         self._last_flags, self._last_Z = flags_dev, Z
         n_nodes = data[DataKey.POSITIONS].shape[0] if DataKey.POSITIONS in data else None
         if self.check_species == "deferred":
diff --git a/matten_amd/ops.py b/matten_amd/ops.py
--- a/matten_amd/ops.py
+++ b/matten_amd/ops.py
@@ -90,7 +90,15 @@
     return err
 
 
-def csr_build(edge_index: torch.Tensor, n_nodes: int, err: torch.Tensor = None) -> Tuple[torch.Tensor, torch.Tensor, torch.Tensor, torch.Tensor]:
+def csr_counters(n_edges: int, n_nodes: int, device) -> Optional[torch.Tensor]:
+    lib = _lib.load()
+    if n_edges <= 0 or n_nodes <= 0 or n_edges > lib.matten_csr_counting_max_avg_degree() * n_nodes:
+        return None
+    return torch.empty(int(lib.matten_csr_counter_words(n_nodes)), dtype=torch.int32, device=device)
+
+
+def csr_build(edge_index: torch.Tensor, n_nodes: int, err: torch.Tensor = None,
+              counters: torch.Tensor = None) -> Tuple[torch.Tensor, torch.Tensor, torch.Tensor, torch.Tensor]:
     lib = _lib.load()
     edge_index = _need(edge_index, torch.int64, "edge_index")
     E = edge_index.shape[1]
@@ -101,9 +109,12 @@
     err = _err_flag(err, dev)
     nbytes = lib.matten_csr_workspace_bytes(E, n_nodes)
     ws = torch.empty(max(nbytes, 1), dtype=torch.uint8, device=dev)
+    if counters is not None and (counters.dtype != torch.int32 or counters.device != dev or not counters.is_contiguous()
+                                 or counters.numel() < lib.matten_csr_counter_words(n_nodes)):
+        raise ValueError("counters must be the int32 tensor csr_counters(n_edges, n_nodes, device) returned")
     _lib.check(
-        lib.matten_csr_build(_ptr(edge_index), E, n_nodes, _ptr(perm), _ptr(rowptr), _ptr(src), _ptr(ws), nbytes,
-                             _ptr(err), _stream()),
+        lib.matten_csr_build_zeroed(_ptr(edge_index), E, n_nodes, _ptr(perm), _ptr(rowptr), _ptr(src), _ptr(ws), nbytes,
+                                    _ptr(err), _ptr(counters), _stream()),
         "matten_csr_build",
     )
     return perm, rowptr, src, err
@@ -141,8 +152,31 @@
     return order, seg, err
 
 
+def group_run_hist(n: int, n_keys: int, device) -> Optional[torch.Tensor]:
+    if not _lib.load().matten_group_self_scan(n, n_keys):
+        return None
+    return torch.empty(n_keys, (n + 63) // 64, dtype=torch.int32, device=device)
+
+
+def group_place(key: torch.Tensor, n_keys: int, run_hist: torch.Tensor, err: torch.Tensor = None):
+    lib = _lib.load()
+    key = _need(key, torch.int64, "key")
+    run_hist = _need(run_hist, torch.int32, "run_hist")
+    n = key.shape[0]
+    dev = key.device
+    if tuple(run_hist.shape) != (n_keys, (n + 63) // 64):
+        raise ValueError(f"run_hist must be [{n_keys}, {(n + 63) // 64}], got {tuple(run_hist.shape)}")
+    order = torch.empty(n, dtype=torch.int32, device=dev)
+    seg = torch.empty(n_keys + 1, dtype=torch.int32, device=dev)
+    err = _err_flag(err, dev)
+    _lib.check(lib.matten_group_place(_ptr(key), n, n_keys, _ptr(run_hist), _ptr(order), _ptr(seg), _ptr(err), _stream()),
+               "matten_group_place")
+    return order, seg, err
+
+
 def species_embed(atomic_numbers, z_to_index, min_z: int, max_z: int, n_species: int, weight, bias,
-                  want_attrs: bool = False, err: torch.Tensor = None):
+                  want_attrs: bool = False, err: torch.Tensor = None, run_hist: torch.Tensor = None,
+                  zero: torch.Tensor = None):
     lib = _lib.load()
     Z = _need(atomic_numbers, torch.int64, "atomic_numbers")
     lut = _need(z_to_index, torch.int64, "_Z_to_index")
@@ -155,9 +189,15 @@
     feats = torch.empty(N, dim, dtype=torch.float32, device=dev)
     attrs = torch.empty(N, n_species, dtype=torch.float32, device=dev) if want_attrs else None
     err = _err_flag(err, dev)
+    if run_hist is not None and (run_hist.dtype != torch.int32 or not run_hist.is_contiguous() or run_hist.device != dev
+                                 or tuple(run_hist.shape) != (n_species, (N + 63) // 64)):
+        raise ValueError("run_hist must be the tensor group_run_hist(N, n_species, device) returned")
+    if zero is not None and (zero.dtype != torch.int32 or not zero.is_contiguous() or zero.device != dev):
+        raise ValueError("zero must be a contiguous int32 tensor on the inputs' device")
     _lib.check(
-        lib.matten_species_embed(_ptr(Z), N, _ptr(lut), min_z, max_z, n_species, _ptr(W), _ptr(b), dim, _ptr(sidx),
-                                 _ptr(s32), _ptr(feats), _ptr(attrs), _ptr(err), _stream()),
+        lib.matten_species_embed_hist(_ptr(Z), N, _ptr(lut), min_z, max_z, n_species, _ptr(W), _ptr(b), dim, _ptr(sidx),
+                                      _ptr(s32), _ptr(feats), _ptr(attrs), _ptr(err), _ptr(run_hist), _ptr(zero),
+                                      0 if zero is None else zero.numel(), _stream()),
         "matten_species_embed",
     )
     return sidx, s32, feats, attrs, err
```
